# timweiland/DiffEqGMRFs.jl

Measured on AMD Instinct MI355X. Metric: GMRF posterior solves/sec (mean+samples), 256^2 Darcy, higher is better.
Workload: dtype f64; 1 GPU; darcy256: n=65536, 64 blocks x 1024, nnz=1624084; 256 independent posterior(s) per GPU and step (4 stream(s) x batch 64), each factor + mean + 64 samples; mode=problems, samples_per_problem_per_rank=64, l_blocks_kept=False

## Files before the change

diffeqgmrfs.jl_amd/_cabi.py:

```python
from __future__ import annotations

import ctypes as C
import os
from typing import Optional

_HERE = os.path.dirname(os.path.abspath(__file__))
LIB_PATH = os.environ.get("GMRF_HIP_LIBRARY") or os.path.join(_HERE, "csrc", "libgmrf_hip.so")

GMRF_OK = 0
ERR_NOT_SPD, ERR_BAD_SHAPE, ERR_BAND, ERR_HIP, ERR_NO_FACTOR, ERR_NO_DEVICE, ERR_ALLOC, ERR_RCCL = -1, -2, -3, -4, -5, -6, -7, -8
SOLVE_FULL, SOLVE_FORWARD, SOLVE_BACKWARD = 0, 1, 2
VAR_EXACT, VAR_RBMC, VAR_MC = 0, 1, 2
BLOCK_L, BLOCK_C, BLOCK_LINV = 0, 1, 2
ORDER_REFERENCE, ORDER_TWISTED = 0, 1

EXPORTS = [
    "gmrf_bt_create", "gmrf_bt_destroy", "gmrf_last_error", "gmrf_version",
    "gmrf_bt_factor_csc", "gmrf_bt_factor_blocks", "gmrf_bt_refactor_values",
    "gmrf_bt_solve", "gmrf_bt_sample", "gmrf_bt_posterior", "gmrf_bt_set_factor_rhs", "gmrf_bt_normals", "gmrf_bt_marginal_var",
    "gmrf_bt_var_accumulate", "gmrf_bt_logdet", "gmrf_bt_get_block", "gmrf_bt_factor_buffer",
    "gmrf_bt_adopt_shape", "gmrf_bt_adopt_commit", "gmrf_bt_adopt_layout", "gmrf_bt_get_layout", "gmrf_bt_block_range",
    "gmrf_bt_set_keep_l", "gmrf_bt_storage_bytes", "gmrf_bt_set_storage", "gmrf_bt_factor_begin_csc",
    "gmrf_bt_factor_step_async", "gmrf_bt_factor_end", "gmrf_bt_stats",
    "gmrf_bt_set_profiling", "gmrf_bt_set_eager", "gmrf_bt_synchronize", "gmrf_bt_set_batch", "gmrf_bt_select_problem",
    "gmrf_bt_marginal_var_batch", "gmrf_bt_selinv", "gmrf_bt_trace_inv", "gmrf_bt_set_order", "gmrf_bt_get_order", "gmrf_bt_half_stats", "gmrf_bt_export_size", "gmrf_bt_export_factor", "gmrf_bt_import_factor",
    "gmrf_comm_unique_id", "gmrf_comm_create", "gmrf_comm_destroy", "gmrf_comm_bcast_host", "gmrf_comm_allreduce_sum",
    "gmrf_bt_bcast_blocks_async", "gmrf_bt_allgather_blocks_async", "gmrf_comm_wait", "gmrf_comm_bytes", "gmrf_streams_create", "gmrf_streams_destroy",
    "gmrf_bt_packed_size", "gmrf_bt_pack_blocks_async", "gmrf_bt_unpack_blocks_async",
    "gmrf_csr_create", "gmrf_csr_destroy", "gmrf_spmm", "gmrf_spmm_rows", "gmrf_spmm_async", "gmrf_spmm_rows_async",
    "gmrf_darcy_p1_create", "gmrf_darcy_p2_create", "gmrf_darcy_p1_destroy", "gmrf_darcy_p1_pattern", "gmrf_darcy_p1_assemble",
    "gmrf_burgers_p1_create", "gmrf_burgers_p2_create", "gmrf_burgers_line_create", "gmrf_burgers_colloc_create", "gmrf_burgers_p1_destroy", "gmrf_burgers_p1_pattern", "gmrf_burgers_p1_tangent",
    "gmrf_shallow_water_p1_create", "gmrf_shallow_water_p1_destroy", "gmrf_shallow_water_p1_pattern", "gmrf_shallow_water_p1_qpoints",
    "gmrf_shallow_water_p1_assemble", "gmrf_shallow_water_p1_operators",
    "gmrf_assemble_create", "gmrf_assemble_destroy", "gmrf_assemble_pattern", "gmrf_assemble_precision", "gmrf_assemble_rhs",
    "gmrf_burgers_p1_tangent_batch", "gmrf_assemble_precision_batch", "gmrf_assemble_rhs_batch", "gmrf_assemble_objective_batch",
    "gmrf_gn_create", "gmrf_gn_destroy", "gmrf_gn_run", "gmrf_gn_finalize",
    "gmrf_elliptic_p1_create", "gmrf_elliptic_p2_create", "gmrf_elliptic_p1_destroy", "gmrf_elliptic_p1_pattern", "gmrf_elliptic_p1_qpoints",
    "gmrf_elliptic_p1_tangent", "gmrf_elliptic_p1_tangent_batch", "gmrf_elliptic_p1_load", "gmrf_gn_create_elliptic",
    "gmrf_darcy_p1_assemble_batch", "gmrf_dc_create", "gmrf_dc_destroy", "gmrf_dc_run",
    "gmrf_burgers_prior_create", "gmrf_burgers_line_prior_create", "gmrf_burgers_prior_destroy", "gmrf_burgers_prior_pattern", "gmrf_burgers_prior_values_batch",
    "gmrf_bic_create", "gmrf_bic_destroy", "gmrf_bic_run", "gmrf_field_errors_batch",
    "gmrf_test_gemm", "gmrf_test_gemm_desc", "gmrf_test_gemm_pair", "gmrf_test_gemm_rate", "gmrf_test_gemm_shapes", "gmrf_test_potrf_tile", "gmrf_test_potrf_block", "gmrf_test_potrf_route", "gmrf_test_tile_timing", "gmrf_test_persist_stamps", "gmrf_test_persist_aborts", "gmrf_test_factor_fwd", "gmrf_test_gn_route", "gmrf_test_dc_route", "gmrf_test_bic_route", "gmrf_test_var_groups", "gmrf_test_persist_budget", "gmrf_test_clock_probe_start", "gmrf_test_clock_probe_finish",
    "gmrf_test_mfma_f64_rate", "gmrf_test_hbm_rate", "gmrf_test_microbench", "gmrf_test_symbolic_csc",
]


class SparseBlock(C.Structure):
    _fields_ = [("nnz", C.c_int64), ("ptr", C.c_void_p), ("idx", C.c_void_p), ("val", C.c_void_p)]


class Stats(C.Structure):
    _fields_ = [
        ("factor_ms", C.c_double), ("solve_ms", C.c_double), ("sample_ms", C.c_double),
        ("factor_flops", C.c_double), ("sweep_bytes", C.c_double), ("sweep_ms", C.c_double),
        ("n", C.c_int64), ("n_blocks", C.c_int64), ("block_size", C.c_int64),
        ("block_size_padded", C.c_int64), ("factor_bytes", C.c_int64),
        ("kernel_ms", C.c_double * 24), ("kernel_work", C.c_double * 24), ("kernel_launches", C.c_int64 * 24),
        ("sweep_bytes_streamed", C.c_double),
        ("persist_route", C.c_int32), ("persist_aborts", C.c_int32), ("persist_cus", C.c_int32), ("persist_refused", C.c_int32),
        ("sweep_persist", C.c_int32), ("sweep_persist_launches", C.c_int32),
    ]


class GmrfError(RuntimeError):
    def __init__(self, status: int, msg: str, info: int = 0):
        super().__init__(f"libgmrf_hip status {status}: {msg}")
        self.status = status
        self.info = info


class NotPositiveDefinite(GmrfError):
    """Julia's PosDefException(info): `.info` is the failing block (1-based)."""


_lib: Optional[C.CDLL] = None


def load() -> C.CDLL:
    global _lib
    if _lib is not None:
        return _lib
    if not os.path.exists(LIB_PATH):
        raise ImportError(
            f"{LIB_PATH} is missing: build it with `python -c 'import __graft_entry__ as g; g.build()'` "
            "or `make -C diffeqgmrfs.jl_amd/csrc` (the HIP library is the only compute path)")
    try:
        import torch
    except Exception:
        pass
    lib = C.CDLL(LIB_PATH)
    vp, i32, i64, u64, dbl = C.c_void_p, C.c_int32, C.c_int64, C.c_uint64, C.c_double
    P = C.POINTER
    sigs = {
        "gmrf_bt_create": [i32, vp, P(vp)],
        "gmrf_bt_destroy": [vp],
        "gmrf_version": [],
        "gmrf_bt_factor_csc": [vp, i64, i64, vp, vp, vp, i32, P(i32)],
        "gmrf_bt_factor_blocks": [vp, i64, i64, vp, vp, i32, i32, P(i32)],
        "gmrf_bt_refactor_values": [vp, vp, P(i32)],
        "gmrf_bt_solve": [vp, vp, vp, i64, i64, i64, i32],
        "gmrf_bt_sample": [vp, u64, i64, i64, vp, vp, vp, i64],
        "gmrf_bt_posterior": [vp, vp, u64, i64, i64, vp, vp, i64],
        "gmrf_bt_set_factor_rhs": [vp, vp],
        "gmrf_bt_normals": [vp, u64, i64, i64, vp, i64],
        "gmrf_bt_marginal_var": [vp, i32, i64, u64, vp, vp],
        "gmrf_bt_var_accumulate": [vp, i32, i64, i64, u64, vp, vp],
        "gmrf_bt_logdet": [vp, P(dbl)],
        "gmrf_bt_get_block": [vp, i32, i64, vp, i64],
        "gmrf_bt_factor_buffer": [vp, i32, P(vp), P(i64)],
        "gmrf_bt_adopt_shape": [vp, i64, i64],
        "gmrf_bt_storage_bytes": [i64, i64, i64, P(i64), P(i64), P(i64)],
        "gmrf_bt_set_storage": [vp, i64, i64, i64, vp, vp, vp],
        "gmrf_bt_adopt_commit": [vp, i32],
        "gmrf_bt_adopt_layout": [vp, i64, i64, vp, i64],
        "gmrf_bt_get_layout": [vp, vp, i64, P(i64)],
        "gmrf_bt_block_range": [vp, i32, i64, i64, P(i64), P(i64), P(i64)],
        "gmrf_bt_set_keep_l": [vp, i32],
        "gmrf_comm_unique_id": [vp],
        "gmrf_comm_create": [i32, i32, i32, vp, P(vp)],
        "gmrf_comm_destroy": [vp],
        "gmrf_comm_bcast_host": [vp, vp, i64, i32],
        "gmrf_comm_allreduce_sum": [vp, vp, vp, i64],
        "gmrf_bt_bcast_blocks_async": [vp, vp, i32, i64, i64, i32],
        "gmrf_bt_allgather_blocks_async": [vp, vp, vp, i64, i64],
        "gmrf_comm_wait": [vp, vp],
        "gmrf_comm_bytes": [vp, i32, P(dbl)],
        "gmrf_bt_packed_size": [vp, i64, i64, P(i64)],
        "gmrf_bt_pack_blocks_async": [vp, i64, i64, vp],
        "gmrf_bt_unpack_blocks_async": [vp, i64, i64, vp],
        "gmrf_streams_create": [i32, i32, vp, vp],
        "gmrf_streams_destroy": [i32, i32, vp],
        "gmrf_bt_factor_begin_csc": [vp, i64, i64, vp, vp, vp, i32],
        "gmrf_bt_factor_step_async": [vp, i64, i64],
        "gmrf_bt_factor_end": [vp, P(i32)],
        "gmrf_bt_stats": [vp, P(Stats)],
        "gmrf_bt_set_order": [vp, i32, i64],
        "gmrf_bt_get_order": [vp, P(i32), P(i64)],
        "gmrf_bt_half_stats": [vp, i32, P(Stats)],
        "gmrf_bt_set_profiling": [vp, i32],
        "gmrf_bt_set_eager": [vp, i32],
        "gmrf_bt_synchronize": [vp],
        "gmrf_bt_set_batch": [vp, i64],
        "gmrf_bt_select_problem": [vp, i64],
        "gmrf_csr_create": [i32, vp, i64, i64, vp, vp, vp, i32, i32, P(vp)],
        "gmrf_bt_marginal_var_batch": [vp, i32, i64, u64, vp, vp, vp],
        "gmrf_bt_selinv": [vp, vp, vp],
        "gmrf_bt_trace_inv": [vp, vp, vp, i64, vp],
        "gmrf_bt_export_size": [vp, P(i64)],
        "gmrf_bt_export_factor": [vp, vp, i64],
        "gmrf_bt_import_factor": [vp, vp, i64],
        "gmrf_csr_destroy": [vp],
        "gmrf_assemble_create": [i32, vp, i64, vp, vp, i64, vp, vp, i32, P(vp)],
        "gmrf_assemble_destroy": [vp],
        "gmrf_assemble_pattern": [vp, P(i64), P(i64), vp, vp, i32],
        "gmrf_assemble_precision": [vp, vp, vp, dbl, vp],
        "gmrf_assemble_rhs": [vp, vp, vp, vp, vp, dbl, vp],
# ... 10 lines not shown
        "gmrf_burgers_p1_pattern": [vp, P(i64), vp, vp, i32],
        "gmrf_burgers_p1_tangent": [vp, vp, vp, vp],
        "gmrf_burgers_p1_tangent_batch": [vp, i64, vp, vp, vp],
        "gmrf_assemble_precision_batch": [vp, i64, vp, i64, vp, dbl, vp],
        "gmrf_assemble_rhs_batch": [vp, i64, vp, vp, vp, vp, dbl, vp],
        "gmrf_assemble_objective_batch": [vp, i64, vp, i64, vp, vp, vp, dbl, vp],
        "gmrf_gn_create": [vp, vp, vp, P(vp)],
        "gmrf_gn_create_elliptic": [vp, vp, vp, P(vp)],
        "gmrf_elliptic_p1_create": [i32, vp, i64, i64, P(vp)],
        "gmrf_elliptic_p2_create": [i32, vp, i64, i64, P(vp)],
        "gmrf_elliptic_p1_destroy": [vp],
        "gmrf_elliptic_p1_pattern": [vp, P(i64), vp, vp, i32],
        "gmrf_elliptic_p1_qpoints": [vp, vp],
        "gmrf_elliptic_p1_tangent": [vp, vp, vp, vp],
        "gmrf_elliptic_p1_tangent_batch": [vp, i64, vp, vp, vp],
        "gmrf_elliptic_p1_load": [vp, i64, vp, vp],
        "gmrf_gn_destroy": [vp],
        "gmrf_gn_run": [vp, vp, i64, vp, vp, vp, vp, dbl, dbl, i32, vp, vp, P(i32)],
        "gmrf_gn_finalize": [vp, P(i32)],
        "gmrf_darcy_p1_assemble_batch": [vp, i64, vp, i64, dbl, vp, vp],
        "gmrf_dc_create": [vp, vp, vp, P(vp)],
        "gmrf_dc_destroy": [vp],
        "gmrf_dc_run": [vp, vp, i64, dbl, vp, i64, vp, dbl, i64, u64, i32, i64, u64, vp, vp, vp, vp, P(i32)],
        "gmrf_burgers_prior_create": [i32, vp, i64, i64, dbl, dbl, dbl, P(vp)],
        "gmrf_burgers_line_prior_create": [i32, vp, i64, i64, dbl, dbl, dbl, i32, i32, dbl, dbl, i32, P(vp)],
        "gmrf_burgers_prior_destroy": [vp],
        "gmrf_burgers_prior_pattern": [vp, P(i64), vp, vp, i32],
        "gmrf_burgers_prior_values_batch": [vp, i64, vp, vp, vp, vp],
        "gmrf_bic_create": [vp, vp, vp, P(vp)],
        "gmrf_bic_destroy": [vp],
        "gmrf_bic_run": [vp, vp, vp, vp, vp, vp, P(i32)],
        "gmrf_field_errors_batch": [i32, vp, i64, i64, i64, vp, vp, vp],
        "gmrf_shallow_water_p1_create": [i32, vp, i64, i64, P(vp)],
        "gmrf_shallow_water_p1_destroy": [vp],
        "gmrf_shallow_water_p1_pattern": [vp, i32, P(i64), vp, vp, i32],
        "gmrf_shallow_water_p1_qpoints": [vp, vp],
        "gmrf_shallow_water_p1_assemble": [vp, vp, dbl, dbl, dbl, vp, vp, vp, vp],
        "gmrf_shallow_water_p1_operators": [vp, vp, vp, vp, vp, dbl, dbl, dbl, vp, vp, vp, vp],
        "gmrf_spmm": [vp, vp, vp, i64, i64, i64],
        "gmrf_spmm_async": [vp, vp, vp, i64, i64, i64],
        "gmrf_spmm_rows_async": [vp, vp, vp, i64, i64, i64],
        "gmrf_spmm_rows": [vp, vp, vp, i64, i64, i64],
        "gmrf_test_gemm": [i32, i64, i64, i64, i32, i32, i32, i32, dbl, vp, i64, vp, i64, dbl, vp, i64],
        "gmrf_test_gemm_shapes": [vp, P(dbl), i64, P(i64)],
        "gmrf_test_gemm_desc": [i32, i32, vp, vp] + [vp, i64] * 12 + [P(i32)],
        "gmrf_test_gemm_pair": [i32, i32, i32, vp, vp, vp, vp, vp, vp, vp, vp],
        "gmrf_test_gemm_rate": [i32, i64, i64, i64, i32, i32, i32, i32, i32, i32, P(dbl)],
        "gmrf_test_potrf_tile": [i32, vp, vp, P(i32)],
        "gmrf_test_potrf_block": [i32, i64, vp, vp, P(i32)],
        "gmrf_test_potrf_route": [i32, i64, i32, i32, i64, i32, vp, vp, vp, P(i32), P(i32)],
        "gmrf_test_tile_timing": [vp, i32],
        "gmrf_test_persist_stamps": [vp, i32],
        "gmrf_test_persist_aborts": [vp, vp],
        "gmrf_test_factor_fwd": [vp, vp, vp],
        "gmrf_test_gn_route": [vp, P(i32), P(i32)],
        "gmrf_test_dc_route": [vp, vp],
        "gmrf_test_bic_route": [vp, vp],
        "gmrf_test_var_groups": [vp, vp, vp],
        "gmrf_test_persist_budget": [i32, i32, vp, vp],
        "gmrf_test_clock_probe_start": [i32, i32, i32, P(vp)],
        "gmrf_test_clock_probe_finish": [vp, vp, vp],
        "gmrf_test_mfma_f64_rate": [i32, P(dbl)],
        "gmrf_test_hbm_rate": [i32, i64, P(dbl)],
        "gmrf_test_microbench": [i32, vp, i32],
        "gmrf_test_symbolic_csc": [i64, i64, vp, vp, i32, vp],
    }
    for name, args in sigs.items():
        fn = getattr(lib, name)
        fn.argtypes = args
        fn.restype = i32
    lib.gmrf_last_error.argtypes = []
    lib.gmrf_last_error.restype = C.c_char_p
    _lib = lib
    return lib


def check(status: int, info: int = 0):
    if status == GMRF_OK:
        return
    msg = load().gmrf_last_error().decode(errors="replace")
    if status == ERR_NOT_SPD:
        raise NotPositiveDefinite(status, msg, info)
    raise GmrfError(status, msg, info)


def ptr(a) -> C.c_void_p:
    if a is None:
        return C.c_void_p(0)
    if isinstance(a, int):
        return C.c_void_p(a)
    if hasattr(a, "data_ptr"):
        return C.c_void_p(a.data_ptr())
    return C.c_void_p(a.ctypes.data)
```

diffeqgmrfs.jl_amd/api.py:

```python
from __future__ import annotations

import ctypes as C
from typing import List, Optional, Sequence, Tuple

import numpy as np
import scipy.sparse as sp

from . import _cabi
from ._cabi import GmrfError, NotPositiveDefinite


def _is_torch(x) -> bool:
    return hasattr(x, "data_ptr") and hasattr(x, "device")


def _colmajor(b, n: int):
    if _is_torch(b):
        import torch
        if b.dtype != torch.float64:
            raise TypeError("float64 required")
        if b.dim() == 1:
            if b.shape[0] != n:
                raise ValueError("dimension mismatch")
            return b.contiguous(), 1, n, True
# ... 1001 lines not shown
        store, view = _alloc_like(like if like is not None else np.empty(0), self.N, k, False)
        _cabi.check(self._lib.gmrf_bt_normals(self._h, seed, first_id, k, _cabi.ptr(store), self.N))
        return view

    def normals_batch(self, k: int, seed: int = 0x5EED, first_id: int = 0):
        out = np.empty((self.batch, k, self.N), dtype=np.float64)
        _cabi.check(self._lib.gmrf_bt_normals(self._h, seed, first_id, k, _cabi.ptr(out), self.N))
        return out

    def sample(self, k: int, mean=None, z=None, seed: int = 0x5EED, first_id: int = 0, like=None):
        ref = like if like is not None else (z if z is not None else (mean if mean is not None else np.empty(0)))
        za = None
        if z is not None:
            za, kz, _, _ = _colmajor(z, self.N)
            k = kz
        if mean is not None and not _is_torch(mean):
            mean = np.ascontiguousarray(mean, dtype=np.float64)
        store, view = _alloc_like(ref if _is_torch(ref) else np.empty(0), self.N, k, False)
        _cabi.check(self._lib.gmrf_bt_sample(self._h, seed, first_id, k, _cabi.ptr(mean), _cabi.ptr(za),
                                             _cabi.ptr(store), self.N))
        return view

    def posterior(self, b, k: int, seed: int = 0x5EED, first_id: int = 0):
        if self.batch != 1:
            raise ValueError("posterior(): one problem per handle (use solve_batch / sample_batch for batches)")
        xa, kb, ld, one_d = _colmajor(b, self.N)
        if kb != 1:
            raise ValueError("posterior(): one right-hand side")
        mstore, mview = _alloc_like(xa, self.N, 1, True)
        sstore, sview = _alloc_like(xa, self.N, k, False)
        _cabi.check(self._lib.gmrf_bt_posterior(self._h, _cabi.ptr(xa), seed, first_id, k, _cabi.ptr(mstore), _cabi.ptr(sstore),
                                                self.N))
        return mview, sview

    def posterior_batch(self, b, k: int, seed: int = 0x5EED, first_id: int = 0):
        import torch
        B, n = self.batch, self.N
        b = b.reshape(B, n).contiguous()
        mean = torch.empty((B, n), dtype=torch.float64, device=b.device)
        out = torch.empty((B, k, n), dtype=torch.float64, device=b.device)
        _cabi.check(self._lib.gmrf_bt_posterior(self._h, _cabi.ptr(b), seed, first_id, k, _cabi.ptr(mean), _cabi.ptr(out), n))
        return mean, out

    def set_factor_rhs(self, b):
        if b is None:
            self._factor_rhs = None
            _cabi.check(self._lib.gmrf_bt_set_factor_rhs(self._h, None))
            return
        if not (_is_torch(b) and b.is_cuda and b.is_contiguous()) or (self.N and b.numel() != self.batch * self.N):
            raise ValueError("set_factor_rhs(): a contiguous device tensor of batch x n values")
        self._factor_rhs = b
        _cabi.check(self._lib.gmrf_bt_set_factor_rhs(self._h, _cabi.ptr(b)))

    def marginal_var(self, method: str = "exact", k: int = 50, seed: int = 0x5EED, Q: Optional[CsrMatrix] = None,
                     q_values=None, out=None):
        m = {"exact": _cabi.VAR_EXACT, "rbmc": _cabi.VAR_RBMC, "mc": _cabi.VAR_MC}[method]
        shape = (self.N,) if self.batch == 1 else (self.batch, self.N)
        if out is None:
            out = np.empty(shape, dtype=np.float64)
        else:
            ok = tuple(out.shape) == shape and (out.is_contiguous() and str(out.dtype) == "torch.float64" if _is_torch(out)
                                                else out.flags.c_contiguous and out.dtype == np.float64)
            if not ok:
                raise ValueError(f"out must be a contiguous float64 array of shape {shape}")
        if self.batch > 1 and m != _cabi.VAR_EXACT:
            qv = None
            if q_values is not None:
                qv = q_values.contiguous() if _is_torch(q_values) else np.ascontiguousarray(q_values, dtype=np.float64)
            _cabi.check(self._lib.gmrf_bt_marginal_var_batch(self._h, m, k, seed, Q._h if Q is not None else None,
                                                             _cabi.ptr(qv) if qv is not None else None, _cabi.ptr(out)))
            return out
        _cabi.check(self._lib.gmrf_bt_marginal_var(self._h, m, k, seed, Q._h if Q is not None else None,
                                                   _cabi.ptr(out)))
        return out

    def selected_inverse(self, S: CsrMatrix, out=None):
        shape = (S.nnz,) if self.batch == 1 else (self.batch, S.nnz)
        given = out is not None
        out = self._out_array(out, shape)
        _cabi.check(self._lib.gmrf_bt_selinv(self._h, S._h, _cabi.ptr(out)))
        if given or self.batch > 1:
            return out
        return sp.csr_matrix((out, S.indices.copy(), S.indptr.copy()), shape=S.shape)

    def trace_inv(self, S: CsrMatrix, dvals):
        nd = 2 if self.batch == 1 else 3
        if dvals.ndim != nd or dvals.shape[-1] != S.nnz or (nd == 3 and dvals.shape[0] != self.batch):
            want = "(m, nnz)" if nd == 2 else "(batch, m, nnz)"
            raise ValueError(f"dvals must be {want} with nnz = {S.nnz}")
        m = int(dvals.shape[-2])
        if _is_torch(dvals):
            import torch
            if dvals.dtype != torch.float64:
                raise TypeError("float64 required")
            dvals = dvals.contiguous()
            out = torch.empty(dvals.shape[:-1], dtype=torch.float64, device=dvals.device)
        else:
            dvals = np.ascontiguousarray(dvals, dtype=np.float64)
            out = np.empty(dvals.shape[:-1], dtype=np.float64)
        _cabi.check(self._lib.gmrf_bt_trace_inv(self._h, S._h, _cabi.ptr(dvals), m, _cabi.ptr(out)))
        return out

    @staticmethod
    def _out_array(out, shape):
        if out is None:
            return np.empty(shape, dtype=np.float64)
# ... 261 lines not shown
```

diffeqgmrfs.jl_amd/csrc/gmrf_hip.hip:

```cpp
#include <hip/hip_runtime.h>
#include <dlfcn.h>
#include <stdint.h>
#include <stdlib.h>
#include <string.h>
#include <time.h>

#include <algorithm>
#include <atomic>
#include <iterator>
#include <cmath>
#include <map>
#include <memory>
#include <chrono>
#include <functional>
#include <initializer_list>
#include <mutex>
#include <string>
#include <type_traits>
#include <vector>

#include "../../include/gmrf_hip.h"
#include "assemble.hpp"
#include "fem_assemble.hpp"
#include "burgers_line.hpp"
// ... 138 lines not shown
    int64_t lo_row_max = 0;
    bool sparse_b = false;
    bool dense_g1 = false;
    double *d_L = nullptr, *d_C = nullptr, *d_Linv = nullptr;
    bool external_storage = false;
    bool keep_l = true;
    bool l_valid = false;
    bool logdet_valid = false;
    std::vector<char> got_block;
    int64_t alloc_rm = 0, alloc_wc = 0;
    bool alloc_keep_l = true;
    double *d_S = nullptr, *d_B = nullptr, *d_T = nullptr, *d_W = nullptr;
    double* d_V = nullptr;
    int64_t v_elems = 0;
    uint64_t layout_gen = 0;
    uint64_t sel_csr = 0, sel_gen = ~0ull;
    int64_t sel_nnz = 0;
    std::vector<int64_t> sel_off, sel_nd;
    int64_t* d_sel_src = nullptr;
    int64_t* d_sel_slot = nullptr;
    int64_t sel_cap = 0;
    double* d_sig = nullptr;
    int64_t sig_elems = 0;
    double* d_dv = nullptr;
    int64_t dv_elems = 0;
    int* d_info = nullptr;
    double* d_logdet = nullptr;
    int64_t alloc_N = 0, alloc_bsp = 0;
    bool factored = false;
    double *d_P = nullptr, *d_Y = nullptr, *d_Tp = nullptr;
    int64_t kp_cap = 0;
    double* d_stage = nullptr;
    int64_t stage_cap = 0;
    DevBuf mean_arena;
    double* d_acc = nullptr;
    int64_t acc_B = 0;
    int32_t var_group = 0, var_groups = 0;
    bool eager = false;
    bool split_step = false;
    bool sweep_no_gemm = false;
    bool no_fused_posterior = false;
    bool tail_probe = false;
    bool tail_refused = false;
    const double* frhs = nullptr;
    const double* fy_for = nullptr;
    bool fwd_run = false;
    bool no_factor_fwd = false;
    bool no_grouped_gemm = false;
    GemmDirectOut* d_dout = nullptr;
    double* d_ft = nullptr;
    double* d_fy = nullptr;
    int64_t fy_elems = 0;
    const double* factor_graph_rhs = nullptr;
    unsigned long long* dbg_stamps = nullptr;
    bool fork_graph = false;
    bool no_staircase = false;
    bool doubling_x = false;
    int xsplit = 0;
    int adopt_xsplit = 0;
    bool no_xsplit = false;
    bool no_lookahead = false;
    bool no_persist = false;
    bool persist_gave_up = false;
    bool persist_launched = false;
    int persist_cus = 0;
    int info_checked = 0;
    int factor_graph_route = 0;
    int persist_aborts = 0;
    int cu_count = 0;
    unsigned* d_pflags = nullptr;
    int64_t pflags_words = 0;
    bool no_sweep_persist = false;
    bool no_scatter_fold = false;
    bool sweep_persist_planned = false;
    bool sweep_persist_launched = false;
    unsigned* d_sweep_flags = nullptr;
    double* d_Tsw = nullptr;
    int64_t t_elems = 0;
    unsigned* h_sweep_abort = nullptr;
    int sweep_nw = 0;
    double *d_P2 = nullptr, *d_Y2 = nullptr, *d_T2 = nullptr;
    int64_t p2_elems = 0;
    bool sweep_persist_hold = false;
    bool no_persist_panels = false;
    hipStream_t aux = nullptr;
    bool aux_distinct = false;
    hipStream_t gemm_stream = nullptr;
    bool capturing = false;
    std::vector<hipEvent_t> fork_events;
    size_t fork_next = 0;
    hipGraphExec_t factor_graph = nullptr;
    int64_t factor_graph_i0 = -1, factor_graph_i1 = -1;
    std::map<int64_t, hipGraphExec_t> sweep_graphs;
    int profiling = 0;
    std::vector<EvPair> events;
    std::vector<hipEvent_t> ev_pool;
    std::vector<GemmShapeStat> gemm_shapes;
    gmrf_stats stats;
    hipEvent_t ev0 = nullptr, ev1 = nullptr;
    int order = GMRF_ORDER_REFERENCE;
    int64_t meet_req = -1;
    int32_t eager_bits = 0;
    TwistState* tw = nullptr;
    int64_t tw_blk = -1;
    const double* tw_hj = nullptr;
    double* tw_w = nullptr;
// ... 311 lines not shown
    HIPCHK(hipMalloc(&h->d_S, blk));
    HIPCHK(hipMalloc(&h->d_B, blk));
    HIPCHK(hipMalloc(&h->d_T, blk));
    HIPCHK(hipMalloc(&h->d_W, blk));
    HIPCHK(hipMalloc(&h->d_logdet, sizeof(double) * h->N * h->B));
    {
        const int64_t words = (int64_t)persist_flag_words((int)(h->bsp / 64)) * h->B;
        if (!h->d_pflags || h->pflags_words < words) {
            free_dev(h->d_pflags); h->d_pflags = nullptr; h->pflags_words = 0;
            HIPCHK(hipMalloc(&h->d_pflags, sizeof(unsigned) * (size_t)words));
            HIPCHK(hipMemsetAsync(h->d_pflags, 0, sizeof(unsigned) * (size_t)words, h->stream));
            HIPCHK(hipStreamSynchronize(h->stream));
            h->pflags_words = words;
        }
    }
    h->alloc_N = h->N; h->alloc_bsp = h->bsp; h->alloc_B = h->B;
    h->stats.factor_bytes = (int64_t)(blk * ((h->keep_l ? 2 : 1) * h->N) + (size_t)stride_pC(h) * sizeof(double) * (size_t)h->B);
    return GMRF_OK;
}

static void release_shape_buffers(gmrf_handle* h) {
    for (auto& kv : h->sweep_graphs) (void)hipGraphExecDestroy(kv.second);
    h->sweep_graphs.clear();
    free_dev(h->d_P); free_dev(h->d_Y); free_dev(h->d_Tp);
    h->d_P = h->d_Y = h->d_Tp = nullptr; h->kp_cap = 0;
    h->mean_arena.release();
    free_dev(h->d_acc); h->d_acc = nullptr; h->acc_B = 0;
    free_dev(h->d_stage); h->d_stage = nullptr; h->stage_cap = 0;
    free_dev(h->d_ft); free_dev(h->d_fy); h->d_ft = h->d_fy = nullptr; h->fy_elems = 0; h->fy_for = nullptr;
}

static gmrf_status set_shape(gmrf_handle* h, int64_t n, int64_t N) {
    if (n <= 0 || N <= 0 || n % N != 0) return bad_shape("n must be a positive multiple of N_blocks");
    const int64_t bs = n / N;
    if (bs > (1 << 20)) return bad_shape("block size too large");
    if (h->n != n || h->N != N) {
        (void)hipStreamSynchronize(h->stream);
        destroy_graphs(h);
        release_shape_buffers(h);
        h->factored = false;
        h->analyzed = false;
    }
    h->n = n; h->N = N; h->bs = bs;
    h->layout_gen++;
    h->bsp = 64 * next_pow2((bs + 63) / 64);
    h->n_pad = h->bsp * N;
    h->stats.n = n; h->stats.n_blocks = N; h->stats.block_size = bs; h->stats.block_size_padded = h->bsp;
    h->stats.factor_flops = ((double)N * bs * bs * bs / 3.0 + (double)(N - 1) * 2.0 * bs * bs * bs) * (double)h->B;
    return GMRF_OK;
}

static gmrf_status ensure_panels(gmrf_handle* h, int64_t kp) {
    if (kp <= h->kp_cap && h->d_P) return GMRF_OK;
    for (auto& kv : h->sweep_graphs) (void)hipGraphExecDestroy(kv.second);
    h->sweep_graphs.clear();
    free_dev(h->d_P); free_dev(h->d_Y); free_dev(h->d_Tp);
    h->d_P = h->d_Y = h->d_Tp = nullptr;
    HIPCHK(hipMalloc(&h->d_P, sizeof(double) * kp * h->n_pad * h->B));
    HIPCHK(hipMalloc(&h->d_Y, sizeof(double) * kp * h->n_pad * h->B));
    HIPCHK(hipMalloc(&h->d_Tp, sizeof(double) * kp * h->bsp * h->B));
    h->kp_cap = kp;
    return GMRF_OK;
}

static gmrf_status ensure_stage(gmrf_handle* h, int64_t elems) {
    if (elems <= h->stage_cap && h->d_stage) return GMRF_OK;
    free_dev(h->d_stage);
    h->d_stage = nullptr;
    HIPCHK(hipMalloc(&h->d_stage, sizeof(double) * elems));
    h->stage_cap = elems;
    return GMRF_OK;
}

struct HostEntry { uint64_t key; int64_t src; };

struct SymbolicPlan {
    std::vector<int64_t> diag_first, diag_count, low_first, low_count;
    std::vector<uint64_t> keys;
    std::vector<int64_t> src;
    int64_t cmin = 0, rmax = 0;
    std::vector<int64_t> first;
    std::vector<int> rowptr;
    int64_t max_row = 0;
    bool sparse_b = false, bxt_ok = false;
    std::vector<int> uptr, ucols, gtiles, ng;
    std::vector<uint16_t> lidx;
    int ecap = 0, nrt = 0;
    std::vector<int> drowptr;
};

static void build_symbolic(int64_t N, int64_t bsp, const std::vector<std::vector<HostEntry>>& dg,
                           const std::vector<std::vector<HostEntry>>& lo, bool no_staircase, SymbolicPlan& sp, bool group_tiles = true) {
    sp.diag_first.assign((size_t)N, 0); sp.diag_count.assign((size_t)N, 0);
    sp.low_first.assign((size_t)N, 0); sp.low_count.assign((size_t)N, 0);
    auto& keys = sp.keys; auto& src = sp.src;
    keys.clear(); src.clear();
    for (int64_t i = 0; i < N; ++i) {
        sp.diag_first[i] = (int64_t)keys.size(); sp.diag_count[i] = (int64_t)dg[i].size();
        {
            std::vector<HostEntry> drow(dg[i]);
            std::stable_sort(drow.begin(), drow.end(), [](const HostEntry& x, const HostEntry& y) { return x.key < y.key; });
            for (auto& e : drow) { keys.push_back(e.key); src.push_back(e.src); }
        }
        sp.low_first[i] = (int64_t)keys.size(); sp.low_count[i] = (int64_t)lo[i].size();
        std::vector<HostEntry> byrow(lo[i]);
        std::stable_sort(byrow.begin(), byrow.end(), [](const HostEntry& x, const HostEntry& y) { return x.key < y.key; });
// ... 340 lines not shown
        }
    }
    h->sweep_persist_planned = ok && want_s > 0 && want >= want_s;
    const int got = ok ? want : 0;
    if (got != h->persist_cus) destroy_graphs(h);
    h->persist_cus = got;
    h->stats.persist_cus = got;
    h->stats.persist_refused = (want > 0 && !ok) ? 1 : 0;
}
static void persist_release(gmrf_handle* h) {
    std::lock_guard<std::mutex> lock(g_persist_mu);
    auto it = g_persist_claims.find(h->device);
    if (it != g_persist_claims.end()) it->second.erase(h);
    h->persist_cus = 0;
    h->stats.persist_cus = 0;
    h->sweep_persist_planned = false;
}

static void persist_give_up(gmrf_handle* h) {
    h->persist_gave_up = true; h->persist_aborts++;
    h->stats.persist_aborts = h->persist_aborts;
    persist_release(h);
    destroy_graphs(h);
}

static bool persist_fits(const gmrf_handle* h, int nt, int j0, int j1, int xrows) {
    if (h->no_persist || h->persist_gave_up || h->persist_cus <= 0) return false;
    return (int64_t)(1 + persist_tiles(nt, j0, j1, xrows)) * h->B <= h->persist_cus;
}

static gmrf_status launch_persist(gmrf_handle* h, double* S, double* L, double* X, int nt, int j0, int j1, int xrows, int blk_id,
                                  double flops) {
    const int words = persist_flag_words(nt);
    if (!h->d_pflags || h->pflags_words < (int64_t)words * h->B) return bad_shape("internal: flag words of the persistent launches not allocated");
    PersistArgs pa;
    pa.S = S; pa.L = L; pa.X = X; pa.ld = h->bsp; pa.nt = nt; pa.j0 = j0; pa.j1 = j1; pa.xrows = xrows;
    pa.tail_panel = (!xrows && j1 < nt) ? 1 : 0;
    pa.info = h->d_info; pa.blk = blk_id;
    pa.pS = h->bsp * h->bsp; pa.pL = stride_pL(h); pa.pX = stride_pX(h); pa.blk_per_problem = (int)h->N;
    pa.flags = h->d_pflags; pa.flag_stride = words;
    pa.abort_word = reinterpret_cast<unsigned*>(h->d_info + 1);
    static const int limit_ms = [] { const char* e = getenv("GMRF_PERSIST_SPIN_MS"); return e ? atoi(e) : -1; }();
    pa.spin_limit = (unsigned)(limit_ms >= 0 ? limit_ms : (h->B > 1 ? 200 : 2000)) * 100000u;
    pa.stamps = h->dbg_stamps;
    h->persist_launched = true;
    h->stats.persist_route = xrows == 1 ? 1 : (xrows == 0 ? 2 : 3);
    ProfScope ps(h, 17, flops);
    hipLaunchKernelGGL(potrf_persist<false>, dim3(1 + persist_tiles(nt, j0, j1, xrows), (unsigned)h->B), dim3(POTRF_PERSIST_THREADS), POTRF_PERSIST_LDS,
                       h->stream, pa);
    HIPCHK(hipGetLastError());
    return GMRF_OK;
}

static gmrf_status potrf_block(gmrf_handle* h, double* S, double* L, double* X, double* T, int blk_id, double* fy = nullptr) {
    const int bsp = (int)h->bsp;
    const int64_t ld = bsp;
    const int nt = bsp / 64;
    const int route = potrf_route(h);
    const bool fused = route == ROUTE_FUSED;
    if (h->xsplit > 0 && route != ROUTE_PANELS256) return bad_shape("internal: split inverse planned off the 256-column panel route");
    static const int pw_env = [] { const char* e = getenv("GMRF_PANEL_TILES"); return e ? atoi(e) : 4; }();
    const int pw = (!fused && nt >= 8) ? ((pw_env == 2 || pw_env == 8) ? pw_env : 4) : nt;
    const bool fused_in_panel = route == ROUTE_BIG_ONE;
    const bool overlap = h->capturing && h->fork_graph && nt >= 8;
    if (overlap && !h->aux) HIPCHK(hipStreamCreateWithFlags(&h->aux, hipStreamNonBlocking));
    hipEvent_t ev_fork = nullptr, ev_join = nullptr;
    if (overlap) { GCHK(fork_event(h, &ev_fork)); GCHK(fork_event(h, &ev_join)); }
    if (fused && !h->no_lookahead && !h->doubling_x && !overlap && nt >= 2 && persist_fits(h, nt, 0, nt, 1)) {
        const double t3 = 64.0 * 64.0 * 64.0;
        double fl = t3 / 3.0 * nt;
        for (int j = 0; j + 1 < nt; ++j) {
            const int m = nt - j - 1;
            fl += (double)m * t3 + 2.0 * t3 * (m * (m + 1) / 2) + 2.0 * t3 * (0.5 * (double)(j + 1) * (j + 2) + 0.625 * (j + 1));
        }
        return launch_persist(h, S, L, X, nt, 0, nt, 1, blk_id, fl);
    }
    if (fused && !h->no_lookahead && !h->doubling_x && !overlap && nt >= 2) {
        StepArgs sa;
        sa.S = S; sa.L = L; sa.X = X; sa.ld = ld; sa.nt = nt; sa.cend = nt;
        sa.info = h->d_info; sa.blk = blk_id; sa.dbg = nullptr;
        sa.pS = (int64_t)bsp * bsp; sa.pL = stride_pL(h); sa.pX = stride_pX(h); sa.blk_per_problem = (int)h->N;
        const double t3 = 64.0 * 64.0 * 64.0;
        {
            sa.j = 0; sa.lookahead = 0; sa.xrow = -1;
            ProfScope ps(h, 1, t3 / 3.0);
            hipLaunchKernelGGL(potrf_step<false>, dim3(1, 1), dim3(256), POTRF_TILE_LDS, h->stream, sa);
        }
        for (int j = 0; j + 1 < nt; ++j) {
            const int m = nt - j - 1, ntile_wg = m * (m + 1) / 2;
            sa.j = j; sa.lookahead = 1;
            sa.xrow = (j >= 1) ? j : -1; sa.xrow_first = ntile_wg;
            const int nx_wg = (j >= 1) ? 4 * j : 0;
            const double f_x = (j >= 1) ? 2.0 * t3 * (0.5 * (double)j * (j + 1) + 0.625 * j) : 0.0;
            ProfScope ps(h, 1, t3 / 3.0 + (double)m * t3 + 2.0 * t3 * ntile_wg + f_x);
            hipLaunchKernelGGL(potrf_step<false>, dim3(ntile_wg + nx_wg, 1), dim3(256), POTRF_STEP_LDS, h->stream, sa);
        }
        {
            sa.j = nt - 1; sa.lookahead = 0; sa.xrow = nt - 1; sa.xrow_first = 0;
            ProfScope ps(h, 1, 2.0 * t3 * (0.5 * (double)(nt - 1) * nt + 0.625 * (nt - 1)));
            hipLaunchKernelGGL(potrf_step<false>, dim3(4 * (nt - 1), 1), dim3(256), 64 * 18 * sizeof(double), h->stream, sa);
        }
        HIPCHK(hipGetLastError());
        return GMRF_OK;
    }
    if (fy && (route != ROUTE_PANELS256 || overlap)) return bad_shape("internal: forward solve planned off the 256-column panel route");
    if (route == ROUTE_PANELS256 && !overlap) {
        StepArgs sa;
        sa.S = S; sa.L = L; sa.X = X; sa.ld = ld; sa.nt = nt; sa.cend = nt;
        sa.info = h->d_info; sa.blk = blk_id; sa.dbg = nullptr;
        sa.pS = (int64_t)bsp * bsp; sa.pL = stride_pL(h); sa.pX = stride_pX(h); sa.blk_per_problem = (int)h->N;
        const int64_t pW = (int64_t)bsp * bsp;
        const double t3 = 64.0 * 64.0 * 64.0, nb = (double)h->B;
        auto diag128 = [&](int j) -> gmrf_status {
            sa.j = j;
            ProfScope ps(h, 16, (2.0 * t3 / 3.0 + 4.0 * 2.0 * t3 * 0.625) * nb);
            static const size_t lds_pad = [] { const char* e = getenv("GMRF_DIAG128_LDS_PAD_KB"); return (size_t)(e ? atoi(e) : 0) * 1024; }();
            static const bool fat = [] { const char* e = getenv("GMRF_DIAG128_FAT"); return e && atoi(e) != 0; }();
            if (fat) hipLaunchKernelGGL(potrf_diag128, dim3(1, (unsigned)h->B), dim3(256), POTRF_DIAG128_LDS + lds_pad, h->stream, sa);
            else hipLaunchKernelGGL(potrf_diag128_slim, dim3(1, (unsigned)h->B), dim3(256), POTRF_DIAG128_SLIM_LDS + lds_pad, h->stream, sa);
            HIPCHK(hipGetLastError());
            return GMRF_OK;
        };
        static const bool no_small = [] { const char* e = getenv("GMRF_PERSIST_PANELS"); return e && atoi(e) == 0; }();
        const bool persist_panels = !no_small && !h->no_persist_panels && persist_fits(h, 4, 0, 4, 2);
        for (int j = 0; j < nt; j += 4) {
            const int64_t oa = (int64_t)j * 64, ob = oa + 128, oc = oa + 256;
            if (persist_panels) {
                const double fl = (4.0 * t3 / 3.0 + 2.0 * t3 * (6.0 * 0.625 + 10.0 + 10.0 + 6.0 * 0.625)) * nb;
                GCHK(launch_persist(h, S + oa * ld + oa, L + oa * ld + oa, X + oa * ld + oa, 4, 0, 4, 2, blk_id, fl));
            } else {
                GCHK(diag128(j));
                GCHK(gemm(h, false, false, 128, 128, 128, TRI_B_UPPER, 0, 1.0, S + ob * ld + oa, ld, X + oa * ld + oa, ld, 0.0, L + ob * ld + oa, ld,
                          sa.pS, sa.pX, sa.pL, 1, 0, 0, 0, nullptr, 0, 0, 0, 2.0 * t3 * 3.0 * 2.0 * nb));
                GCHK(gemm_pair(h,
                               GemmOne{false, 128, 128, 128, 0, 1, -1.0, L + ob * ld + oa, ld, L + ob * ld + oa, ld, 1.0, S + ob * ld + ob, ld,
                                       sa.pL, sa.pL, sa.pS, 2.0 * t3 * 2.0 * 3.0 * nb},
                               GemmOne{true, 128, 128, 128, TRI_B_LOWER, 0, 1.0, L + ob * ld + oa, ld, X + oa * ld + oa, ld, 0.0, T + ob * ld + oa, ld,
                                       sa.pL, sa.pX, pW, -1.0}));
                GCHK(diag128(j + 2));
                GCHK(gemm(h, false, true, 128, 128, 128, TRI_A_LOWER, 0, -1.0, X + ob * ld + ob, ld, T + ob * ld + oa, ld, 0.0, X + ob * ld + oa, ld,
                          sa.pX, pW, sa.pX));
            }
            const int m3 = nt - j - 4;
            const int64_t pT = bsp, pY = h->n_pad;
            if (m3 <= 0) {
                if (fy) {
                    SweepArgs sw;
                    sw.Mat = X + oa * ld + oa; sw.ld = ld; sw.Xin = h->d_ft + oa; sw.ldx = pT; sw.Bin = nullptr; sw.ldb = 0;
                    sw.Out = fy + oa; sw.ldo = pY; sw.rows = 256; sw.kdim = 256; sw.sub = 0;
                    sw.pMat = sa.pX; sw.pXin = pT; sw.pBin = 0; sw.pOut = pY;
                    ProfScope ps(h, 3, 4.0 * 256.0 * 257.0 * nb);
                    HIPCHK(launch_sweep(h->stream, false, true, 1, sw, (int)h->B));
                }
                continue;
            }
            const GemmTail tp{h->d_ft + oa, pT, fy + oa, pY, nullptr, 0, 0.0};
            const GemmTail tu{fy + oa, pY, h->d_ft + oc, pT, nullptr, 0, 1.0};
            const bool in_slot = (j == 0 && h->xsplit == 256 && !h->keep_l);
            double* Lb = in_slot ? X + oc * ld + oa : L + oc * ld + oa;
            const int64_t pLb = in_slot ? sa.pX : sa.pL;
            GCHK(gemm(h, false, false, 64 * m3, 256, 256, TRI_B_UPPER, 0, 1.0, S + oc * ld + oa, ld, X + oa * ld + oa, ld, 0.0, Lb, ld,
                      sa.pS, sa.pX, pLb, 1, 0, 0, 0, nullptr, 0, 0, 0, 2.0 * t3 * 10.0 * m3 * nb, nullptr, nullptr, nullptr, false,
                      fy ? &tp : nullptr));
            GCHK(gemm(h, false, false, m3 * 64, m3 * 64, 256, 0, 1, -1.0, Lb, ld, Lb, ld, 1.0, S + oc * ld + oc, ld, pLb, pLb, sa.pS,
                      1, 0, 0, 0, nullptr, 0, 0, 0, 2.0 * t3 * 4.0 * (m3 * (m3 + 1) / 2) * nb, nullptr, nullptr, nullptr, false,
                      fy ? &tu : nullptr));
        }
        const int p = h->xsplit;
        GCHK(doubling_levels(h, L, X, T, 256, bsp / 2, -1, p));
        if (p > 0 && !(p == 256 && !h->keep_l)) {
            hipLaunchKernelGGL(copy_rect, dim3((unsigned)((bsp - p) / 4), (unsigned)h->B), dim3(256), 0, h->stream,
                               L + (int64_t)p * ld, ld, sa.pL, X + (int64_t)p * ld, ld, sa.pX, bsp - p, p);
            HIPCHK(hipGetLastError());
        }
        return GMRF_OK;
    }
    if (h->xsplit > 0) return bad_shape("internal: split inverse planned off the 256-column panel route");
// ... 227 lines not shown
    const int bsp = (int)h->bsp, p = h->xsplit, q = bsp - p;
    const int64_t ld = bsp, bstride = (int64_t)bsp * bsp, pX = stride_pX(h), pW = bstride;
    for (int64_t i = 0; i < h->N; ++i) {
        double* X = h->d_Linv + i * bstride;
        double* T = h->d_T + (int64_t)p * ld;
        GCHK(gemm(h, false, true, q, p, p, TRI_B_LOWER, 0, 1.0, X + (int64_t)p * ld, ld, X, ld, 0.0, T, ld, pX, pX, pW));
        GCHK(gemm(h, false, true, q, p, q, TRI_A_LOWER, 0, -1.0, X + (int64_t)p * ld + p, ld, T, ld, 0.0, X + (int64_t)p * ld, ld, pX, pW, pX));
    }
    h->xsplit = 0;
    return GMRF_OK;
}

static std::mutex g_capture_mu;

static gmrf_status factor_fwd_ok(gmrf_handle* h, bool* ok) {
    *ok = false;
    if (!h->frhs || h->no_factor_fwd || h->B <= 1 || tw_on(h) || h->tw_blk >= 0 || h->fork_graph || h->rmax <= 0) return GMRF_OK;
    const int bsp = (int)h->bsp, nt = bsp / 64;
    if (potrf_route(h) != ROUTE_PANELS256 || bsp % 256 != 0) return GMRF_OK;
    const int64_t elems = h->B * h->n_pad + h->B * h->bsp;
    if (!h->d_fy || h->fy_elems < elems) {
        HIPCHK(hipStreamSynchronize(h->stream));
        free_dev(h->d_ft); free_dev(h->d_fy); h->d_ft = h->d_fy = nullptr; h->fy_elems = 0; h->fy_for = nullptr;
        HIPCHK(hipMalloc(&h->d_fy, sizeof(double) * (size_t)(h->B * h->n_pad)));
        HIPCHK(hipMalloc(&h->d_ft, sizeof(double) * (size_t)(h->B * h->bsp)));
        h->fy_elems = elems;
    }
    const int64_t ld = bsp, bstride = (int64_t)bsp * bsp, pX = stride_pX(h), pL = stride_pL(h), pC = stride_pC(h);
    const int cm = (int)h->cmin, rm = (int)h->rmax, W = bsp - cm;
    double* S = h->d_S; double* X = h->d_Linv; double* L = h->d_L;
    h->tail_probe = true; h->tail_refused = false;
    gmrf_status st = GMRF_OK;
    if (h->N > 1) {
        const GemmTail tg{h->d_fy + cm, h->n_pad, h->d_ft, bsp, nullptr, 0, 1.0};
        st = gemm(h, false, false, rm, rm, W, 0, 1, -1.0, h->d_C, c_ld(h), h->d_C, c_ld(h), 0.0, S, ld, pC, pC, bstride, 1, 0, 0, 0,
                  nullptr, 0, 0, 0, -1.0, h->d_kst, h->d_kst, nullptr, false, &tg);
    }
    for (int j = 0; j + 4 < nt && st == GMRF_OK; j += 4) {
        const int64_t oa = (int64_t)j * 64, oc = oa + 256;
        const int m3 = nt - j - 4;
        const GemmTail tp{h->d_ft + oa, bsp, h->d_fy + oa, h->n_pad, nullptr, 0, 0.0};
        const GemmTail tu{h->d_fy + oa, h->n_pad, h->d_ft + oc, bsp, nullptr, 0, 1.0};
        st = gemm(h, false, false, 64 * m3, 256, 256, TRI_B_UPPER, 0, 1.0, S + oc * ld + oa, ld, X + oa * ld + oa, ld, 0.0, L + oc * ld + oa, ld,
                  bstride, pX, pL, 1, 0, 0, 0, nullptr, 0, 0, 0, -1.0, nullptr, nullptr, nullptr, false, &tp);
        if (st == GMRF_OK)
            st = gemm(h, false, false, m3 * 64, m3 * 64, 256, 0, 1, -1.0, L + oc * ld + oa, ld, L + oc * ld + oa, ld, 1.0, S + oc * ld + oc, ld,
                      pL, pL, bstride, 1, 0, 0, 0, nullptr, 0, 0, 0, -1.0, nullptr, nullptr, nullptr, false, &tu);
    }
    h->tail_probe = false;
    *ok = st == GMRF_OK && !h->tail_refused;
    return GMRF_OK;
}

static gmrf_status run_factor(gmrf_handle* h, int64_t i0, int64_t i1) {
    if (h->eager || h->profiling) { h->stats.persist_route = 0; return factor_blocks_range(h, i0, i1); }
    const double* grhs = h->fwd_run ? h->frhs : nullptr;
    if (!h->factor_graph || h->factor_graph_i0 != i0 || h->factor_graph_i1 != i1 || h->factor_graph_rhs != grhs) {
        std::lock_guard<std::mutex> capture_lock(g_capture_mu);
        if (h->factor_graph) { (void)hipGraphExecDestroy(h->factor_graph); h->factor_graph = nullptr; }
        hipGraph_t graph = nullptr;
        HIPCHK(hipStreamBeginCapture(h->stream, hipStreamCaptureModeThreadLocal));
        h->capturing = true; h->fork_next = 0;
        h->stats.persist_route = 0;
        gmrf_status s = factor_blocks_range(h, i0, i1);
        h->capturing = false;
        h->factor_graph_route = h->stats.persist_route;
        hipError_t e = hipStreamEndCapture(h->stream, &graph);
        if (s != GMRF_OK) { if (graph) (void)hipGraphDestroy(graph); return s; }
        HIPCHK(e);
        HIPCHK(hipGraphInstantiate(&h->factor_graph, graph, nullptr, nullptr, 0));
        (void)hipGraphDestroy(graph);
        h->factor_graph_i0 = i0; h->factor_graph_i1 = i1; h->factor_graph_rhs = grhs;
    }
    h->xsplit = planned_xsplit(h);
    h->stats.persist_route = h->factor_graph_route;
    if (h->factor_graph_route) h->persist_launched = true;
    HIPCHK(hipGraphLaunch(h->factor_graph, h->stream));
    return GMRF_OK;
}

static gmrf_status persist_check_range(gmrf_handle* h, int64_t i0, int64_t i1, int* hinfo_out) {
    int hinfo2[2] = {0, 0};
    HIPCHK(hipMemcpyAsync(hinfo2, h->d_info, 2 * sizeof(int), hipMemcpyDeviceToHost, h->stream));
    HIPCHK(hipStreamSynchronize(h->stream));
    h->persist_launched = false;
    if (hinfo2[1] != 0) {
        persist_give_up(h);
        const int restore[4] = {h->info_checked, 0, 0, 0};
        HIPCHK(hipMemcpyAsync(h->d_info, restore, 4 * sizeof(int), hipMemcpyHostToDevice, h->stream));
        if (h->d_pflags) HIPCHK(hipMemsetAsync(h->d_pflags, 0, sizeof(unsigned) * (size_t)h->pflags_words, h->stream));
        h->stats.persist_route = 0;
        GCHK(factor_blocks_range(h, i0, i1));
        HIPCHK(hipMemcpyAsync(hinfo2, h->d_info, 2 * sizeof(int), hipMemcpyDeviceToHost, h->stream));
        HIPCHK(hipStreamSynchronize(h->stream));
        h->persist_launched = false;
    }
    h->info_checked = hinfo2[0];
    if (hinfo_out) *hinfo_out = hinfo2[0];
    return GMRF_OK;
}

static gmrf_status factor_finish(gmrf_handle* h, int32_t* info) {
    int hinfo = 0;
    GCHK(persist_check_range(h, 0, h->N, &hinfo));
    if (info) *info = hinfo;
    if (hinfo != 0) {
        h->factored = false;
        g_last_error = "matrix is not positive definite; failed block " + std::to_string((hinfo - 1) % h->N + 1) +
                       " of problem " + std::to_string((hinfo - 1) / h->N);
        if (info) *info = (hinfo - 1) % (int)h->N + 1;
        return GMRF_ERR_NOT_SPD;
    }
    h->factored = true;
    h->l_valid = h->keep_l;
    h->logdet_valid = !h->keep_l;
    return GMRF_OK;
}

static gmrf_status numeric_factor(gmrf_handle* h, const double* nzval, int32_t* info) {
    if (!h->analyzed) { g_last_error = "no sparsity pattern analysed"; return GMRF_ERR_NO_FACTOR; }
    GCHK(alloc_factor(h));
    if (h->c_dirty) {
        HIPCHK(hipMemsetAsync(h->d_C, 0, sizeof(double) * stride_pC(h) * h->B, h->stream));
        h->c_dirty = false;
    }
    persist_plan(h);
    HIPCHK(hipEventRecord(h->ev0, h->stream));
    GCHK(load_values(h, nzval));
    HIPCHK(hipMemsetAsync(h->d_info, 0, 4 * sizeof(int), h->stream));
    h->info_checked = 0; h->persist_launched = false;
    h->fy_for = nullptr;
    bool fwd = false;
    GCHK(factor_fwd_ok(h, &fwd));
    h->fwd_run = fwd;
    gmrf_status s = run_factor(h, 0, h->N);
    if (s == GMRF_OK) {
        (void)hipEventRecord(h->ev1, h->stream);
        s = factor_finish(h, info);
    }
    h->fwd_run = false;
    if (s == GMRF_OK && fwd) h->fy_for = h->frhs;
    float ms = 0.f;
    (void)hipEventElapsedTime(&ms, h->ev0, h->ev1);
    h->stats.factor_ms = ms;
    if (h->profiling) prof_collect(h);
    return s;
}

__global__ void gmrf_spin_kernel(unsigned long long ticks) {
    const unsigned long long t0 = __builtin_amdgcn_s_memrealtime();
    while (__builtin_amdgcn_s_memrealtime() - t0 < ticks) {}
}

static double spin_pair_ms(hipStream_t a, hipStream_t b, unsigned long long ticks) {
    (void)hipDeviceSynchronize();
    const auto t0 = std::chrono::steady_clock::now();
    hipLaunchKernelGGL(gmrf_spin_kernel, dim3(1), dim3(64), 0, a, ticks);
    if (b) hipLaunchKernelGGL(gmrf_spin_kernel, dim3(1), dim3(64), 0, b, ticks);
    (void)hipStreamSynchronize(a);
    if (b) (void)hipStreamSynchronize(b);
    return std::chrono::duration<double, std::milli>(std::chrono::steady_clock::now() - t0).count();
}

gmrf_status gmrf_streams_create(int32_t device, int32_t n, void** streams, int32_t* n_distinct) {
    if (n <= 0 || n > 32 || !streams) return bad_shape("gmrf_streams_create: 1 <= n <= 32 streams");
    HIPCHK(hipSetDevice(device));
    const int ncand = std::min(3 * n + 4, 48);
    std::vector<hipStream_t> cand((size_t)ncand, nullptr);
    for (int i = 0; i < ncand; ++i) {
        if (hipStreamCreateWithFlags(&cand[(size_t)i], hipStreamNonBlocking) != hipSuccess) {
            for (int j = 0; j < i; ++j) (void)hipStreamDestroy(cand[(size_t)j]);
            g_last_error = "hipStreamCreateWithFlags failed"; return GMRF_ERR_HIP;
        }
        hipLaunchKernelGGL(gmrf_spin_kernel, dim3(1), dim3(64), 0, cand[(size_t)i], 1ull);
    }
    HIPCHK(hipDeviceSynchronize());
    const unsigned long long ticks = 100000ull;
    double one = 1e30;
    for (int r = 0; r < 3; ++r) one = std::min(one, spin_pair_ms(cand[0], nullptr, ticks));
    std::vector<int> chosen;
    for (int i = 0; i < ncand && (int)chosen.size() < n; ++i) {
        bool ok = true;
        for (int c : chosen) {
            const double t = std::min(spin_pair_ms(cand[(size_t)c], cand[(size_t)i], ticks), spin_pair_ms(cand[(size_t)c], cand[(size_t)i], ticks));
            if (t > 1.5 * one) { ok = false; break; }
        }
        if (ok) chosen.push_back(i);
    }
    const int nd = (int)chosen.size();
    std::vector<char> used((size_t)ncand, 0);
    for (int c : chosen) used[(size_t)c] = 1;
    for (int i = 0; i < ncand && (int)chosen.size() < n; ++i)
        if (!used[(size_t)i]) { chosen.push_back(i); used[(size_t)i] = 1; }
    for (int k = 0; k < n; ++k) streams[k] = (void*)cand[(size_t)chosen[(size_t)k]];
// ... 163 lines not shown
        double* yout = Yout + i * bsp;
        auto direct = [&](int first) { return GemmTail{nullptr, 0, nullptr, 0, nullptr, 0, 0.0, dout, i * h->bs + first, (int)h->bs - first}; };
        if (h->xsplit > 0) {
            const int p = h->xsplit, q = bsp - p;
            const double* Xbb = X + (int64_t)p * ld + p;
            const double* Lba = X + (int64_t)p * ld;
            for (int part = 0; part < 3; ++part) {
                const int which = backward ? 2 - part : part;
                if (via_gemm) {
                    constexpr int64_t z0 = 0;
                    const GemmTail da = direct(0), db = direct(p);
                    if (which == 0)
                        GCHK(gemm(h, false, backward, kp, p, p, backward ? TRI_B_LOWER : TRI_B_UPPER, 0, 1.0, rhs, npad, X, ld, 0.0, yout, npad,
                                  pPanel, pX, pPanel, 1, z0, z0, z0, nullptr, z0, z0, 0, -1.0, nullptr, nullptr, nullptr, tail,
                                  dout ? &da : nullptr));
                    else if (which == 2)
                        GCHK(gemm(h, false, backward, kp, q, q, backward ? TRI_B_LOWER : TRI_B_UPPER, 0, 1.0, rhs + p, npad, Xbb, ld, 0.0,
                                  yout + p, npad, pPanel, pX, pPanel, 1, z0, z0, z0, nullptr, z0, z0, 0, -1.0, nullptr, nullptr, nullptr, tail,
                                  dout ? &db : nullptr));
                    else if (!backward)
                        GCHK(gemm(h, false, false, kp, q, p, 0, 0, -1.0, yout, npad, Lba, ld, 1.0, rhs + p, npad, pPanel, pX, pPanel));
                    else
                        GCHK(gemm(h, false, true, kp, p, q, 0, 0, -1.0, yout + p, npad, Lba, ld, 1.0, rhs, npad, pPanel, pX, pPanel,
                                  1, z0, z0, z0, nullptr, z0, z0, 0, -1.0, nullptr, nullptr, nullptr, tail));
                } else {
                    s.ld = ld; s.ldx = npad; s.ldo = npad; s.pMat = pX; s.pXin = pPanel; s.pOut = pPanel; s.kst = nullptr; s.mend = nullptr;
                    if (which == 0) { s.Mat = X; s.Xin = rhs; s.Bin = nullptr; s.ldb = 0; s.Out = yout; s.rows = p; s.kdim = p; s.sub = 0; s.pBin = 0; }
                    else if (which == 2) { s.Mat = Xbb; s.Xin = rhs + p; s.Bin = nullptr; s.ldb = 0; s.Out = yout + p; s.rows = q; s.kdim = q; s.sub = 0; s.pBin = 0; }
                    else if (!backward) { s.Mat = Lba; s.Xin = yout; s.Bin = rhs + p; s.ldb = npad; s.Out = rhs + p; s.rows = q; s.kdim = p; s.sub = 1; s.pBin = pPanel; }
                    else { s.Mat = Lba; s.Xin = yout + p; s.Bin = rhs; s.ldb = npad; s.Out = rhs; s.rows = p; s.kdim = q; s.sub = 1; s.pBin = pPanel; }
                    const double frac = which == 0 ? (double)p * (p + 1) : (which == 2 ? (double)q * (q + 1) : 2.0 * p * q);
                    ProfScope ps(h, pclass, blk_work_t * frac / ((double)bsp * (bsp + 1)));
                    HIPCHK(launch_sweep(h->stream, backward, which != 1, kp, s, nprob));
                }
            }
        } else if (via_gemm) {
            const GemmTail da = direct(0);
            GCHK(gemm(h, false, backward, kp, bsp, bsp, backward ? TRI_B_LOWER : TRI_B_UPPER, 0, 1.0, rhs, npad, X, ld, 0.0,
                      yout, npad, pPanel, pX, pPanel, 1, 0, 0, 0, nullptr, 0, 0, 0, -1.0, nullptr, nullptr, nullptr, tail, dout ? &da : nullptr));
        } else {
            s.Mat = X; s.ld = ld; s.Xin = rhs; s.ldx = npad; s.Bin = nullptr; s.ldb = 0; s.Out = yout; s.ldo = npad;
            s.rows = bsp; s.kdim = bsp; s.sub = 0;
            s.pMat = pX; s.pXin = pPanel; s.pBin = 0; s.pOut = pPanel;
            s.kst = nullptr; s.mend = nullptr;
            ProfScope ps(h, pclass, blk_work_t);
            HIPCHK(launch_sweep(h->stream, backward, true, kp, s, nprob));
        }
    }
    return GMRF_OK;
}

constexpr int SWEEP_BACKWARD_YP = 3, SWEEP_BACKWARD_TAIL = 4;
static gmrf_status run_sweeps(gmrf_handle* h, int mode, int kp) {
    auto body = [&]() -> gmrf_status {
        if (mode == GMRF_SOLVE_FORWARD) return sweep_launches(h, false, kp, h->d_P, h->d_Y);
        if (mode == SWEEP_BACKWARD_TAIL) return sweep_launches(h, true, kp, h->d_P, h->d_Y, true, h->d_dout);
        if (mode == SWEEP_BACKWARD_YP) return sweep_launches(h, true, kp, h->d_Y, h->d_P);
        if (mode == GMRF_SOLVE_BACKWARD) return sweep_launches(h, true, kp, h->d_P, h->d_Y);
        GCHK(sweep_launches(h, false, kp, h->d_P, h->d_Y));
        return sweep_launches(h, true, kp, h->d_Y, h->d_P);
    };
    const bool persistent = mode != SWEEP_BACKWARD_TAIL && sweep_persist_ok(h, kp);
    if (persistent) {
        GCHK(sweep_persist_prepare(h, kp));
        h->sweep_persist_launched = true;
        h->stats.sweep_persist = 1;
        h->stats.sweep_persist_launches += (mode == GMRF_SOLVE_FULL) ? 2 : 1;
    }
    if (h->eager || h->profiling) return body();
    const int64_t key = ((int64_t)h->xsplit << 32) | ((int64_t)mode * 4096 + kp) |
                        (persistent ? ((int64_t)1 << 60) : 0);
    auto it = h->sweep_graphs.find(key);
    if (it == h->sweep_graphs.end()) {
        std::lock_guard<std::mutex> capture_lock(g_capture_mu);
        hipGraph_t graph = nullptr;
        hipGraphExec_t exec = nullptr;
        HIPCHK(hipStreamBeginCapture(h->stream, hipStreamCaptureModeThreadLocal));
        gmrf_status s = body();
        hipError_t e = hipStreamEndCapture(h->stream, &graph);
        if (s != GMRF_OK) { if (graph) (void)hipGraphDestroy(graph); return s; }
        HIPCHK(e);
        HIPCHK(hipGraphInstantiate(&exec, graph, nullptr, nullptr, 0));
        (void)hipGraphDestroy(graph);
        it = h->sweep_graphs.emplace(key, exec).first;
    }
    HIPCHK(hipGraphLaunch(it->second, h->stream));
    return GMRF_OK;
}

static int pad_k(int64_t k) { return k == 1 ? 1 : (int)((k + 15) / 16 * 16); }

static gmrf_status launch_pack(gmrf_handle* h, const double* d_src, int64_t ld, int k, int kp) {
    const int64_t total = (int64_t)kp * h->n_pad;
    hipLaunchKernelGGL(pack_panel, dim3((unsigned)((total + 255) / 256), (unsigned)h->B), dim3(256), 0, h->stream, d_src, ld,
                       h->d_P, h->n_pad, (int)h->bs, (int)h->bsp, (int)h->N, k, kp);
    HIPCHK(hipGetLastError());
    return GMRF_OK;
}

static gmrf_status launch_unpack(gmrf_handle* h, const double* panel, double* d_dst, int64_t ld, int k,
                                 const double* d_mean) {
    const int64_t total = h->n * (int64_t)k;
    hipLaunchKernelGGL(unpack_panel, dim3((unsigned)((total + 255) / 256), (unsigned)h->B), dim3(256), 0, h->stream, panel,
                       h->n_pad, d_dst, ld, (int)h->bs, (int)h->bsp, h->n, k, pad_k(k), d_mean);
    HIPCHK(hipGetLastError());
    return GMRF_OK;
}

static gmrf_status cols_in(gmrf_handle* h, const double* src, int64_t ld, bool src_dev, int k, const double** d_src, int64_t* d_ld) {
    *d_src = src; *d_ld = ld;
    if (src_dev) return GMRF_OK;
    GCHK(ensure_stage(h, (int64_t)k * h->n * h->B));
    HIPCHK(hipMemcpy2DAsync(h->d_stage, h->n * sizeof(double), src, ld * sizeof(double),
                            h->n * sizeof(double), k * h->B, hipMemcpyHostToDevice, h->stream));
    *d_src = h->d_stage; *d_ld = h->n;
    return GMRF_OK;
}

static gmrf_status cols_out(gmrf_handle* h, const double* panel, int k, const double* d_mean, double* dst, int64_t ld, bool dst_dev) {
    if (dst_dev) return launch_unpack(h, panel, dst, ld, k, d_mean);
    GCHK(ensure_stage(h, (int64_t)k * h->n * h->B));
    GCHK(launch_unpack(h, panel, h->d_stage, h->n, k, d_mean));
    HIPCHK(hipMemcpy2DAsync(dst, ld * sizeof(double), h->d_stage, h->n * sizeof(double),
                            h->n * sizeof(double), k * h->B, hipMemcpyDeviceToHost, h->stream));
    return GMRF_OK;
}

constexpr int64_t KP_CHUNK = 128;

static void tw_free(gmrf_handle* h);
static gmrf_status tw_analyze(gmrf_handle* h, int64_t n, int64_t N, const int64_t* colptr, const int64_t* rowval, int32_t base);
static gmrf_status tw_numeric(gmrf_handle* h, const double* nzval, int32_t* info);
static gmrf_status tw_solve(gmrf_handle* h, const double* b, double* y, int64_t k, int64_t ldb, int64_t ldy, int mode);
static gmrf_status tw_sample(gmrf_handle* h, uint64_t seed, int64_t first_id, int64_t k, const double* mean, const double* z,
                             double* out, int64_t ld);
static gmrf_status tw_logdet(gmrf_handle* h, double* out);
static gmrf_status tw_get_block(gmrf_handle* h, int32_t kind, int64_t i, double* out, int64_t ld);
static gmrf_status tw_var_exact(gmrf_handle* h, double* d_out);
static gmrf_status tw_var_accumulate_dev(gmrf_handle* h, int method, int64_t first_id, int64_t k, uint64_t seed, const gmrf_csr* Q,
                                         double* d_acc);

extern "C" {

int32_t gmrf_version(void) { return 100; }
const char* gmrf_last_error(void) { return g_last_error.c_str(); }

gmrf_status gmrf_bt_create(int32_t device, void* stream, gmrf_handle** out) {
    if (!out) return bad_shape("null out pointer");
    int count = 0;
    if (hipGetDeviceCount(&count) != hipSuccess || count <= 0 || device < 0 || device >= count) {
        (void)hipGetLastError();
        g_last_error = "no HIP device visible (libgmrf_hip needs an MI355X / gfx950 GPU)";
        return GMRF_ERR_NO_DEVICE;
    }
    HIPCHK(hipSetDevice(device));
    gmrf_handle* h = new gmrf_handle();
    memset(&h->stats, 0, sizeof(h->stats));
    h->device = device;
    if (stream) { h->stream = (hipStream_t)stream; h->own_stream = false; }
    else { HIPCHK(hipStreamCreateWithFlags(&h->stream, hipStreamNonBlocking)); h->own_stream = true; }
    HIPCHK(hipMalloc(&h->d_info, 4 * sizeof(int)));
    HIPCHK(hipMemsetAsync(h->d_info, 0, 4 * sizeof(int), h->stream));
    HIPCHK(hipStreamSynchronize(h->stream));
    HIPCHK(hipEventCreate(&h->ev0));
    HIPCHK(hipEventCreate(&h->ev1));
    HIPCHK(hipFuncSetAttribute((const void*)potrf_step<false>, hipFuncAttributeMaxDynamicSharedMemorySize, (int)POTRF_STEP_LDS));
    HIPCHK(hipFuncSetAttribute((const void*)potrf_diag128, hipFuncAttributeMaxDynamicSharedMemorySize, 160 * 1024));
    HIPCHK(hipFuncSetAttribute((const void*)potrf_persist<false>, hipFuncAttributeMaxDynamicSharedMemorySize, (int)POTRF_PERSIST_LDS));
    HIPCHK(hipDeviceGetAttribute(&h->cu_count, hipDeviceAttributeMultiprocessorCount, device));
    { const char* e = getenv("GMRF_PERSIST"); if (e && atoi(e) == 0) h->no_persist = true; }
    { const char* e = getenv("GMRF_SWEEP_PERSIST"); if (e && atoi(e) == 0) h->no_sweep_persist = true; }
    HIPCHK(hipFuncSetAttribute((const void*)potrf_diag128_slim, hipFuncAttributeMaxDynamicSharedMemorySize, 160 * 1024));
    HIPCHK(gemm_init());
    HIPCHK(gemm_dma_init());
    *out = h;
    return GMRF_OK;
}

gmrf_status gmrf_bt_destroy(gmrf_handle* h) {
    if (!h) return GMRF_OK;
    (void)hipSetDevice(h->device);
    tw_free(h);
    (void)hipStreamSynchronize(h->stream);
    persist_release(h);
    destroy_graphs(h);
    free_dev(h->d_keys); free_dev(h->d_vals); free_dev(h->d_src); free_dev(h->d_nz_stage);
    free_dev(h->d_lo_rowptr); free_dev(h->d_dg_rowptr); free_dev(h->d_kst); free_dev(h->d_mend);
    free_dev(h->d_bxt_uptr); free_dev(h->d_bxt_ucols); free_dev(h->d_bxt_lidx); free_dev(h->d_bxt_gtiles);
    if (!h->external_storage) { free_dev(h->d_L); free_dev(h->d_C); free_dev(h->d_Linv); }
    else if (!h->keep_l) free_dev(h->d_L);
    free_dev(h->d_S); free_dev(h->d_B); free_dev(h->d_T); free_dev(h->d_W);
    free_dev(h->d_sweep_flags); free_dev(h->d_Tsw); free_dev(h->d_P2); free_dev(h->d_Y2); free_dev(h->d_T2);
    if (h->h_sweep_abort) { (void)hipHostFree(h->h_sweep_abort); h->h_sweep_abort = nullptr; }
    free_dev(h->d_dout); free_dev(h->d_info); free_dev(h->d_logdet); free_dev(h->d_pflags); free_dev(h->d_kbx); free_dev(h->d_V);
    free_dev(h->d_P); free_dev(h->d_Y); free_dev(h->d_Tp);
    free_dev(h->d_stage); h->mean_arena.release(); free_dev(h->d_acc);
    free_dev(h->d_ft); free_dev(h->d_fy);
    free_dev(h->d_sel_src); free_dev(h->d_sel_slot); free_dev(h->d_sig); free_dev(h->d_dv);
    for (auto e : h->ev_pool) (void)hipEventDestroy(e);
    if (h->ev0) (void)hipEventDestroy(h->ev0);
    if (h->ev1) (void)hipEventDestroy(h->ev1);
    for (auto e : h->fork_events) (void)hipEventDestroy(e);
    if (h->aux) (void)hipStreamDestroy(h->aux);
    if (h->own_stream) (void)hipStreamDestroy(h->stream);
    delete h;
    return GMRF_OK;
}

gmrf_status gmrf_bt_set_batch(gmrf_handle* h, int64_t batch) {
    if (!h || batch < 1 || batch > 4096) return bad_shape("batch must be in [1, 4096]");
    if (batch != 1) GCHK(tw_refuse(h, "gmrf_bt_set_batch (batch > 1)"));
    if (batch != h->B) {
        HIPCHK(hipSetDevice(h->device));
        HIPCHK(hipStreamSynchronize(h->stream));
        destroy_graphs(h);
        h->B = batch;
        h->sel = 0;
        h->factored = false;
        release_shape_buffers(h);
        if (h->n > 0) (void)set_shape(h, h->n, h->N);
    }
    return GMRF_OK;
}

gmrf_status gmrf_bt_select_problem(gmrf_handle* h, int64_t p) {
    if (!h || p < 0 || p >= h->B) return bad_shape("problem index out of range");
    h->sel = p;
    return GMRF_OK;
}

gmrf_status gmrf_bt_set_profiling(gmrf_handle* h, int32_t level) {
    if (!h) return bad_shape("null handle");
    h->profiling = level;
    if (h->tw)
        for (gmrf_handle* s : {h->tw->top, h->tw->bot}) if (s) GCHK(gmrf_bt_set_profiling(s, level));
    if (level > 0 && h->events.empty()) h->gemm_shapes.clear();
    for (int i = 0; i < GMRF_KERNEL_CLASSES; ++i) { h->stats.kernel_ms[i] = h->stats.kernel_work[i] = 0; h->stats.kernel_launches[i] = 0; }
    return GMRF_OK;
}

gmrf_status gmrf_bt_set_eager(gmrf_handle* h, int32_t eager) {
    if (!h) return bad_shape("null handle");
    if (((eager & 2) != 0) != h->split_step) { destroy_graphs(h); h->split_step = (eager & 2) != 0; }
    if (((eager & 4) != 0) != h->sweep_no_gemm) { destroy_graphs(h); h->sweep_no_gemm = (eager & 4) != 0; }
    if (((eager & 8) != 0) != h->dense_g1) { destroy_graphs(h); h->dense_g1 = (eager & 8) != 0; }
    if (((eager & 16) != 0) != h->fork_graph) { destroy_graphs(h); h->fork_graph = (eager & 16) != 0; }
    h->no_staircase = (eager & 32) != 0;
    if (((eager & 128) != 0) != h->doubling_x) { destroy_graphs(h); h->doubling_x = (eager & 128) != 0; }
    if (((eager & 256) != 0) != h->no_lookahead) { destroy_graphs(h); h->no_lookahead = (eager & 256) != 0; }
    if (((eager & 4096) != 0) != h->no_xsplit) { destroy_graphs(h); h->no_xsplit = (eager & 4096) != 0; }
    if (((eager & 8192) != 0) != h->no_persist) { destroy_graphs(h); h->no_persist = (eager & 8192) != 0; }
    if (((eager & 32768) != 0) != h->no_persist_panels) { destroy_graphs(h); h->no_persist_panels = (eager & 32768) != 0; }
    if (((eager & 65536) != 0) != h->no_sweep_persist) { destroy_graphs(h); h->no_sweep_persist = (eager & 65536) != 0; }
    if (((eager & 131072) != 0) != h->no_scatter_fold) { destroy_graphs(h); h->no_scatter_fold = (eager & 131072) != 0; }
    h->no_fused_posterior = (eager & 262144) != 0;
    h->no_factor_fwd = (eager & 524288) != 0;
    if (((eager & 1048576) != 0) != h->no_grouped_gemm) { destroy_graphs(h); h->no_grouped_gemm = (eager & 1048576) != 0; }
    if (eager != h->eager_bits) h->fy_for = nullptr;
    h->eager = (eager & 1) != 0;
    h->eager_bits = eager;
    if (h->tw)
        for (gmrf_handle* s : {h->tw->top, h->tw->bot})
            if (s) {
                GCHK(gmrf_bt_set_eager(s, eager));
                if (h->tw->bot) s->no_sweep_persist = true;
            }
    return GMRF_OK;
}

gmrf_status gmrf_bt_synchronize(gmrf_handle* h) {
    if (!h) return bad_shape("null handle");
    HIPCHK(hipStreamSynchronize(h->stream));
    if (tw_on(h)) HIPCHK(hipStreamSynchronize(h->tw->bot->stream));
    return GMRF_OK;
}

gmrf_status gmrf_bt_stats(gmrf_handle* h, gmrf_stats* out) {
    if (!h || !out) return bad_shape("null pointer");
    if (tw_on(h)) {
        const gmrf_stats &a = h->tw->top->stats, &b = h->tw->bot->stats;
        *out = h->stats;
        out->persist_route = a.persist_route;
        out->persist_aborts = a.persist_aborts + b.persist_aborts;
        out->persist_cus = a.persist_cus + b.persist_cus;
        out->persist_refused = a.persist_refused | b.persist_refused;
        out->factor_bytes = a.factor_bytes + b.factor_bytes;
        return GMRF_OK;
    }
    h = tw_route(h);
    *out = h->stats;
    return GMRF_OK;
}

gmrf_status gmrf_bt_factor_csc(gmrf_handle* h, int64_t n, int64_t n_blocks, const int64_t* colptr,
                               const int64_t* rowval, const double* nzval, int32_t index_base,
                               int32_t* info) {
    if (!h) return bad_shape("null handle");
    HIPCHK(hipSetDevice(h->device));
    if (info) *info = 0;
    if (h->order == GMRF_ORDER_TWISTED) {
        GCHK(tw_analyze(h, n, n_blocks, colptr, rowval, index_base));
        return tw_numeric(h, nzval, info);
    }
    GCHK(analyze_csc(h, n, n_blocks, colptr, rowval, index_base));
    return numeric_factor(h, nzval, info);
}

gmrf_status gmrf_bt_factor_begin_csc(gmrf_handle* h, int64_t n, int64_t n_blocks, const int64_t* colptr,
                                     const int64_t* rowval, const double* nzval, int32_t index_base) {
    GCHK(tw_refuse(h, "gmrf_bt_factor_begin_csc"));
    if (!h) return bad_shape("null handle");
    HIPCHK(hipSetDevice(h->device));
    if (colptr) GCHK(analyze_csc(h, n, n_blocks, colptr, rowval, index_base));
    if (!h->analyzed) { g_last_error = "no sparsity pattern analysed"; return GMRF_ERR_NO_FACTOR; }
    GCHK(alloc_factor(h));
    if (h->c_dirty) {
        HIPCHK(hipMemsetAsync(h->d_C, 0, sizeof(double) * stride_pC(h) * h->B, h->stream));
        h->c_dirty = false;
    }
    persist_plan(h);
    GCHK(load_values(h, nzval));
    HIPCHK(hipMemsetAsync(h->d_info, 0, 4 * sizeof(int), h->stream));
    h->info_checked = 0; h->persist_launched = false; h->stats.persist_route = 0;
    h->factored = false; h->fy_for = nullptr;
    return GMRF_OK;
}

gmrf_status gmrf_bt_factor_step_async(gmrf_handle* h, int64_t i0, int64_t i1) {
    GCHK(tw_refuse(h, "gmrf_bt_factor_step_async"));
    if (!h) return bad_shape("null handle");
    if (i0 < 0 || i1 > h->N || i0 > i1) return bad_shape("bad block range");
    HIPCHK(hipSetDevice(h->device));
    GCHK(factor_blocks_range(h, i0, i1));
    if (h->persist_launched) GCHK(persist_check_range(h, i0, i1, nullptr));
    return GMRF_OK;
}

gmrf_status gmrf_bt_factor_end(gmrf_handle* h, int32_t* info) {
    GCHK(tw_refuse(h, "gmrf_bt_factor_end"));
    if (!h) return bad_shape("null handle");
    HIPCHK(hipSetDevice(h->device));
    gmrf_status s = factor_finish(h, info);
    if (h->profiling) prof_collect(h);
    return s;
}

gmrf_status gmrf_bt_refactor_values(gmrf_handle* h, const double* nzval, int32_t* info) {
    if (!h) return bad_shape("null handle");
    HIPCHK(hipSetDevice(h->device));
    if (info) *info = 0;
    if (h->order == GMRF_ORDER_TWISTED) return tw_numeric(h, nzval, info);
    return numeric_factor(h, nzval, info);
}

gmrf_status gmrf_bt_factor_blocks(gmrf_handle* h, int64_t n, int64_t n_blocks, const gmrf_sparse_block* diag,
                                  const gmrf_sparse_block* lower, int32_t index_base,
                                  int32_t compressed_by_column, int32_t* info) {
    GCHK(tw_refuse(h, "gmrf_bt_factor_blocks"));
    if (!h || !diag || (n_blocks > 1 && !lower)) return bad_shape("null pointer");
    HIPCHK(hipSetDevice(h->device));
    if (info) *info = 0;
    GCHK(set_shape(h, n, n_blocks));
    const int64_t bs = h->bs;
    std::vector<std::vector<HostEntry>> dg(n_blocks), lo(n_blocks);
    std::vector<double> vals;
    auto add_block = [&](const gmrf_sparse_block& b, std::vector<HostEntry>& dst, bool lower_tri_only) -> bool {
        for (int64_t o = 0; o < bs; ++o) {
            for (int64_t p = b.ptr[o] - index_base; p < b.ptr[o + 1] - index_base; ++p) {
                const int64_t in = b.idx[p] - index_base;
                if (in < 0 || in >= bs) return false;
                const int64_t r = compressed_by_column ? in : o, c = compressed_by_column ? o : in;
                if (lower_tri_only && r < c) continue;
                dst.push_back({((uint64_t)r << 32) | (uint64_t)c, (int64_t)vals.size()});
                vals.push_back(b.val[p]);
            }
        }
        return true;
// ... 75 lines not shown
    for (int64_t t = 0; t < nrt; ++t) out[3 + t] = h->kst[(size_t)t];
    out[3 + nrt] = h->factored ? h->xsplit : planned_xsplit(h);
    return GMRF_OK;
}

gmrf_status gmrf_bt_adopt_layout(gmrf_handle* h, int64_t n, int64_t n_blocks, const int64_t* layout, int64_t count) {
    GCHK(tw_refuse(h, "gmrf_bt_adopt_layout"));
    if (!h) return bad_shape("null handle");
    HIPCHK(hipSetDevice(h->device));
    GCHK(set_shape(h, n, n_blocks));
    h->analyzed = false;
    if (layout) {
        if (count < 3 || layout[2] < 1 || count < 3 + layout[2] || layout[1] != 64 * layout[2]) return bad_shape("bad layout record");
        std::vector<int64_t> first((size_t)layout[2]);
        for (int64_t t = 0; t < layout[2]; ++t) first[(size_t)t] = layout[0] + layout[3 + t];
        GCHK(set_layout(h, layout[0], layout[1], first));
        h->adopt_xsplit = 0;
        if (count >= 4 + layout[2]) {
            const int64_t xs = layout[3 + layout[2]];
            if (xs < 0 || xs >= h->bsp || xs % 64) return bad_shape("bad layout record (split)");
            h->adopt_xsplit = (int)xs;
        }
    } else {
        GCHK(set_layout_dense(h));
        h->adopt_xsplit = 0;
    }
    GCHK(alloc_factor(h));
    if (h->c_dirty) {
        HIPCHK(hipMemsetAsync(h->d_C, 0, sizeof(double) * stride_pC(h) * h->B, h->stream));
        h->c_dirty = false;
    }
    h->factored = false; h->l_valid = false; h->logdet_valid = false;
    h->got_block.assign((size_t)h->N, 0);
    HIPCHK(hipStreamSynchronize(h->stream));
    return GMRF_OK;
}

gmrf_status gmrf_bt_adopt_shape(gmrf_handle* h, int64_t n, int64_t n_blocks) {
    GCHK(tw_refuse(h, "gmrf_bt_adopt_shape"));
    return gmrf_bt_adopt_layout(h, n, n_blocks, nullptr, 0);
}

gmrf_status gmrf_bt_adopt_commit(gmrf_handle* h, int32_t l_blocks_valid) {
    GCHK(tw_refuse(h, "gmrf_bt_adopt_commit"));
    if (!h || !h->d_Linv) return bad_shape("no factor storage");
    HIPCHK(hipSetDevice(h->device));
    int seen = 0;
    HIPCHK(hipMemcpyAsync(&seen, h->d_info + 2, sizeof(int), hipMemcpyDeviceToHost, h->stream));
    HIPCHK(hipStreamSynchronize(h->stream));
    if (seen != 0) HIPCHK(hipMemsetAsync(h->d_info + 2, 0, sizeof(int), h->stream));
    if (seen < 0) { g_last_error = "the packed ranges of this factor carry different (or no) representation tags"; return GMRF_ERR_BAD_SHAPE; }
    const int xs = seen > 0 ? seen - 1 : h->adopt_xsplit;
    if (xs < 0 || xs >= h->bsp || xs % 64) { g_last_error = "bad representation tag in the packed image"; return GMRF_ERR_BAD_SHAPE; }
    h->factored = true; h->fy_for = nullptr;
    h->xsplit = xs;
    h->l_valid = l_blocks_valid != 0 && h->keep_l;
    bool all = !h->got_block.empty();
    for (char g : h->got_block) all = all && g;
    h->logdet_valid = all;
    h->got_block.assign((size_t)h->N, 0);
    persist_plan(h);
    return GMRF_OK;
}

gmrf_status gmrf_bt_factor_buffer(gmrf_handle* h, int32_t kind, void** dev_ptr, int64_t* bytes) {
    GCHK(tw_refuse(h, "gmrf_bt_factor_buffer"));
    if (!h || !dev_ptr || !bytes) return bad_shape("null pointer");
    if (!h->d_Linv) { g_last_error = "no factor storage"; return GMRF_ERR_NO_FACTOR; }
    const int64_t blk = blk_elems(h) * (int64_t)sizeof(double) * h->B;
    if (kind == GMRF_BLOCK_L) {
        if (!h->keep_l) { g_last_error = "L blocks are not kept (gmrf_bt_set_keep_l)"; return GMRF_ERR_NO_FACTOR; }
        *dev_ptr = h->d_L; *bytes = blk * h->N;
    }
    else if (kind == GMRF_BLOCK_C) { *dev_ptr = h->d_C; *bytes = stride_pC(h) * (int64_t)sizeof(double) * h->B; }
    else if (kind == GMRF_BLOCK_LINV) { *dev_ptr = h->d_Linv; *bytes = blk * h->N; }
    else return bad_shape("bad block kind");
    return GMRF_OK;
}

gmrf_status gmrf_bt_block_range(gmrf_handle* h, int32_t kind, int64_t i0, int64_t i1, int64_t* first_elem,
                                int64_t* n_elems, int64_t* problem_stride) {
    GCHK(tw_refuse(h, "gmrf_bt_block_range"));
    if (!h || !first_elem || !n_elems || !problem_stride) return bad_shape("null pointer");
    if (h->N <= 0 || i0 < 0 || i1 > h->N || i0 > i1) return bad_shape("bad block range");
    if (kind == GMRF_BLOCK_C) {
        const int64_t c0 = std::max<int64_t>(i0 - 1, 0), c1 = std::max<int64_t>(i1 - 1, 0);
        *first_elem = c0 * c_blk(h); *n_elems = (c1 - c0) * c_blk(h); *problem_stride = stride_pC(h);
    } else if (kind == GMRF_BLOCK_LINV || kind == GMRF_BLOCK_L) {
        if (kind == GMRF_BLOCK_L && !h->keep_l) { g_last_error = "L blocks are not kept"; return GMRF_ERR_NO_FACTOR; }
        *first_elem = i0 * blk_elems(h); *n_elems = (i1 - i0) * blk_elems(h);
        *problem_stride = kind == GMRF_BLOCK_L ? stride_pL(h) : stride_pX(h);
    } else return bad_shape("bad block kind");
    return GMRF_OK;
}

static void packed_counts(const gmrf_handle* h, int64_t i0, int64_t i1, int64_t* x_elems, int64_t* c_elems, int64_t* ld_elems,
                          int64_t* c0_out) {
    const int64_t nt = h->bsp / 64, ntri = nt * (nt + 1) / 2;
    const int64_t c0 = std::max<int64_t>(i0 - 1, 0), c1 = std::max<int64_t>(i1 - 1, 0);
    *x_elems = (i1 - i0) * ntri * 4096;
    *c_elems = (c1 - c0) * c_blk(h);
    *ld_elems = 2 + ((i1 - i0) + 1) / 2 * 2;
    if (c0_out) *c0_out = c0;
}

gmrf_status gmrf_bt_packed_size(gmrf_handle* h, int64_t i0, int64_t i1, int64_t* elems_per_problem) {
    GCHK(tw_refuse(h, "gmrf_bt_packed_size"));
// ... 133 lines not shown
    for (int64_t i = 0; i < h->N; ++i) GCHK(gmrf_bt_get_block(h, GMRF_BLOCK_LINV, i, out + i * be, h->bs));
    return GMRF_OK;
}

gmrf_status gmrf_bt_import_factor(gmrf_handle* h, const void* buf, int64_t bytes) {
    GCHK(tw_refuse(h, "gmrf_bt_import_factor"));
    if (!h || !buf) return bad_shape("null pointer");
    if (is_device_ptr(buf)) return bad_shape("import buffer must be host memory");
    if (bytes < 64) return bad_shape("import buffer too small");
    const int64_t* hdr = (const int64_t*)buf;
    if (hdr[0] != EXPORT_MAGIC || hdr[1] != 1 || hdr[5] != 1) return bad_shape("not a factor image");
    const int64_t n = hdr[2], N = hdr[3], bs = hdr[4];
    if (N <= 0 || bs <= 0 || n != N * bs) return bad_shape("bad shape in factor image");
    if (bytes < 64 + (int64_t)sizeof(double) * bs * bs * (3 * N - 1)) return bad_shape("factor image truncated");
    HIPCHK(hipSetDevice(h->device));
    if (!h->keep_l) return bad_shape("import needs the L blocks kept (gmrf_bt_set_keep_l(h, 1))");
    if ((h->n != n || h->N != N) && h->B != 1) return bad_shape("a batched handle imports into an existing shape only");
    const bool relayout = (h->n != n || h->N != N || h->cmin != 0 || h->rmax != 64 * next_pow2((bs + 63) / 64) || !h->d_Linv);
    if (relayout && h->B != 1 && h->factored) return bad_shape("a batched handle imports only into a dense-layout factor");
    GCHK(set_shape(h, n, N));
    h->analyzed = false;
    if (relayout) {
        GCHK(set_layout_dense(h));
        GCHK(alloc_factor(h));
        if (h->c_dirty) {
            HIPCHK(hipMemsetAsync(h->d_C, 0, sizeof(double) * stride_pC(h) * h->B, h->stream));
            h->c_dirty = false;
        }
    } else {
        std::vector<int64_t> z((size_t)(h->bsp / 64), 0);
        bool dense_ks = true;
        for (int v : h->kst) if (v != 0) dense_ks = false;
        if (!dense_ks) GCHK(set_layout(h, 0, h->bsp, z));
        h->c_dirty = false;
    }
    const int64_t bsp = h->bsp, be = bs * bs;
    std::vector<double> tmp((size_t)bsp * bsp);
    auto put = [&](const double* src, double* dst, bool unit_pad) -> gmrf_status {
        std::fill(tmp.begin(), tmp.end(), 0.0);
        for (int64_t r = 0; r < bs; ++r)
            for (int64_t c = 0; c < bs; ++c) tmp[(size_t)r * bsp + c] = src[c * bs + r];
        if (unit_pad)
            for (int64_t r = bs; r < bsp; ++r) tmp[(size_t)r * bsp + r] = 1.0;
        HIPCHK(hipMemcpyAsync(dst, tmp.data(), tmp.size() * sizeof(double), hipMemcpyHostToDevice, h->stream));
        HIPCHK(hipStreamSynchronize(h->stream));
        return GMRF_OK;
    };
    const double* in = (const double*)((const char*)buf + 64);
    for (int64_t i = 0; i < N; ++i) GCHK(put(in + i * be, h->d_L + h->sel * stride_pL(h) + i * blk_elems(h), true));
    in += N * be;
    for (int64_t i = 0; i + 1 < N; ++i) GCHK(put(in + i * be, h->d_C + h->sel * stride_pC(h) + i * c_blk(h), false));
    in += (N - 1) * be;
    for (int64_t i = 0; i < N; ++i) GCHK(put(in + i * be, h->d_Linv + h->sel * stride_pX(h) + i * blk_elems(h), true));
    h->factored = true; h->fy_for = nullptr; h->l_valid = true;
    persist_plan(h);
    h->xsplit = 0;
    return GMRF_OK;
}

struct NcclUid { char b[128]; };
struct RcclApi {
    void* lib = nullptr;
    int (*GetUniqueId)(NcclUid*) = nullptr;
    int (*CommInitRank)(void**, int, NcclUid, int) = nullptr;
    int (*CommDestroy)(void*) = nullptr;
    int (*Broadcast)(const void*, void*, size_t, int, int, void*, hipStream_t) = nullptr;
    int (*AllReduce)(const void*, void*, size_t, int, int, void*, hipStream_t) = nullptr;
    int (*AllGather)(const void*, void*, size_t, int, void*, hipStream_t) = nullptr;
    int (*GroupStart)() = nullptr;
    int (*GroupEnd)() = nullptr;
    const char* (*GetErrorString)(int) = nullptr;
};
static RcclApi g_rccl;
static std::mutex g_rccl_mu;

static gmrf_status rccl_load() {
    std::lock_guard<std::mutex> lock(g_rccl_mu);
    if (g_rccl.lib) return GMRF_OK;
    const char* env = getenv("GMRF_RCCL_PATH");
    const char* names[] = {env, "librccl.so.1", "librccl.so", "/opt/rocm/lib/librccl.so.1", "/opt/rocm/lib/librccl.so"};
    void* lib = nullptr;
    for (int pass = 0; pass < 2 && !lib; ++pass)
        for (const char* nm : names) {
            if (!nm) continue;
            lib = dlopen(nm, RTLD_NOW | RTLD_LOCAL | (pass == 0 ? RTLD_NOLOAD : 0));
            if (lib) break;
        }
    if (!lib) { g_last_error = std::string("librccl not found (set GMRF_RCCL_PATH): ") + (dlerror() ? dlerror() : ""); return GMRF_ERR_RCCL; }
#define GMRF_RCCL_SYM(field, name)                                                           \
    g_rccl.field = reinterpret_cast<decltype(g_rccl.field)>(dlsym(lib, name));               \
    if (!g_rccl.field) { g_last_error = std::string("librccl lacks ") + name; return GMRF_ERR_RCCL; }
    GMRF_RCCL_SYM(GetUniqueId, "ncclGetUniqueId") GMRF_RCCL_SYM(CommInitRank, "ncclCommInitRank")
    GMRF_RCCL_SYM(CommDestroy, "ncclCommDestroy") GMRF_RCCL_SYM(Broadcast, "ncclBroadcast")
    GMRF_RCCL_SYM(AllReduce, "ncclAllReduce") GMRF_RCCL_SYM(AllGather, "ncclAllGather") GMRF_RCCL_SYM(GroupStart, "ncclGroupStart")
    GMRF_RCCL_SYM(GroupEnd, "ncclGroupEnd") GMRF_RCCL_SYM(GetErrorString, "ncclGetErrorString")
#undef GMRF_RCCL_SYM
    g_rccl.lib = lib;
    return GMRF_OK;
}

#define NCCLCHK(expr)                                                                       \
    do {                                                                                    \
        int _r = (expr);                                                                    \
        if (_r != 0) {                                                                      \
            g_last_error = std::string(#expr) + ": " + g_rccl.GetErrorString(_r);           \
            return GMRF_ERR_RCCL;                                                           \
        }                                                                                   \
// ... 162 lines not shown
}

gmrf_status gmrf_bt_solve(gmrf_handle* h, const double* b, double* y, int64_t k, int64_t ldb, int64_t ldy, int32_t mode) {
    h = tw_route(h);
    if (!h || !b || !y) return bad_shape("null pointer");
    if (!h->factored) { g_last_error = "solve before factor"; return GMRF_ERR_NO_FACTOR; }
    if (k <= 0 || ldb < h->n || ldy < h->n || mode < 0 || mode > 2) return bad_shape("bad k / ldb / ldy / mode");
    if (b == y && ldb != ldy) return bad_shape("in place (y == b) needs ldb == ldy");
    HIPCHK(hipSetDevice(h->device));
    if (tw_on(h)) return tw_solve(h, b, y, k, ldb, ldy, mode);
    if (h->B > 1 && k > KP_CHUNK) return bad_shape("with a batch of problems k is limited to 128 per call");
    const bool b_dev = is_device_ptr(b), y_dev = is_device_ptr(y);
    const int64_t nb = h->B;
    return sweep_guarded(h, {{b, cols_bytes(h->n, k * nb, ldb), y, cols_bytes(h->n, k * nb, ldy)}}, [&]() -> gmrf_status {
        h->stats.solve_ms = 0.0;
        for (int64_t c0 = 0; c0 < k; c0 += KP_CHUNK) {
            const int kc = (int)std::min<int64_t>(KP_CHUNK, k - c0);
            const int kp = pad_k(kc);
            GCHK(ensure_panels(h, kp));
            const double* d_b = nullptr;
            int64_t ld_b = 0;
            GCHK(cols_in(h, b + c0 * ldb, ldb, b_dev, kc, &d_b, &ld_b));
            GCHK(launch_pack(h, d_b, ld_b, kc, kp));
            HIPCHK(hipEventRecord(h->ev0, h->stream));
            GCHK(run_sweeps(h, mode, kp));
            HIPCHK(hipEventRecord(h->ev1, h->stream));
            GCHK(cols_out(h, (mode == GMRF_SOLVE_FULL) ? h->d_P : h->d_Y, kc, nullptr, y + c0 * ldy, ldy, y_dev));
            HIPCHK(hipStreamSynchronize(h->stream));
            float ms = 0.f;
            (void)hipEventElapsedTime(&ms, h->ev0, h->ev1);
            h->stats.solve_ms += ms;
            const int nsweeps = (mode == GMRF_SOLVE_FULL) ? 2 : 1;
            h->stats.sweep_ms = ms / nsweeps;
            h->stats.sweep_bytes = sweep_bytes(h, kc) * (double)nb;
            h->stats.sweep_bytes_streamed = (8.0 * ((double)h->N * 0.5 * (double)h->bsp * (double)(h->bsp + 1) +
                                                    (double)(h->N - 1) * h->c_streamed) + 16.0 * (double)h->n_pad * kc) * (double)nb;
            if (h->profiling) prof_collect(h);
        }
        return GMRF_OK;
    });
}

static gmrf_status sample_chunk(gmrf_handle* h, uint64_t seed, int64_t first_id, int kc, const double* z,
                                int64_t ldz, int64_t id_stride) {
    const int kp = pad_k(kc);
    GCHK(ensure_panels(h, kp));
    if (z) {
        const double* d_z = nullptr;
        int64_t ldd = 0;
        GCHK(cols_in(h, z, ldz, is_device_ptr(z), kc, &d_z, &ldd));
        GCHK(launch_pack(h, d_z, ldd, kc, kp));
    } else {
        const int64_t total = (int64_t)kp * h->n_pad;
        hipLaunchKernelGGL(fill_normals_panel, dim3((unsigned)((total + 255) / 256), (unsigned)h->B), dim3(256), 0,
                           h->stream, h->d_P, h->n_pad, (int)h->bs, (int)h->bsp, kc, kp, seed, first_id, id_stride, nullptr, (int64_t)0);
        HIPCHK(hipGetLastError());
    }
    return run_sweeps(h, GMRF_SOLVE_BACKWARD, kp);
}

gmrf_status gmrf_bt_sample(gmrf_handle* h, uint64_t seed, int64_t first_id, int64_t k, const double* mean,
                           const double* z, double* out, int64_t ld) {
    h = tw_route(h);
    if (!h || !out) return bad_shape("null pointer");
    if (!h->factored) { g_last_error = "sample before factor"; return GMRF_ERR_NO_FACTOR; }
    if (k <= 0 || ld < h->n) return bad_shape("bad k / ld");
    if (h->B > 1 && k > KP_CHUNK) return bad_shape("with a batch of problems k is limited to 128 per call");
    HIPCHK(hipSetDevice(h->device));
    if (tw_on(h)) return tw_sample(h, seed, first_id, k, mean, z, out, ld);
    const double* d_mean = nullptr;
    Staging args(h->mean_arena);
    args.in(mean, sizeof(double) * h->n * h->B, &d_mean);
    GCHK(args.commit(h->stream));
    const bool out_dev = is_device_ptr(out);
    const int64_t smp_bytes = cols_bytes(h->n, k * h->B, ld);
    GCHK(sweep_guarded(h, {{z, smp_bytes, out, smp_bytes}, {mean, h->n * h->B * (int64_t)sizeof(double), out, smp_bytes}},
                       [&]() -> gmrf_status {
        HIPCHK(hipEventRecord(h->ev0, h->stream));
        for (int64_t c0 = 0; c0 < k; c0 += KP_CHUNK) {
            const int kc = (int)std::min<int64_t>(KP_CHUNK, k - c0);
            GCHK(sample_chunk(h, seed, first_id + c0, kc, z ? z + c0 * ld : nullptr, ld, k));
            GCHK(cols_out(h, h->d_Y, kc, d_mean, out + c0 * ld, ld, out_dev));
            if (!out_dev) HIPCHK(hipStreamSynchronize(h->stream));
        }
        HIPCHK(hipEventRecord(h->ev1, h->stream));
        HIPCHK(hipStreamSynchronize(h->stream));
        return GMRF_OK;
    }));
    float ms = 0.f;
    (void)hipEventElapsedTime(&ms, h->ev0, h->ev1);
    h->stats.sample_ms = ms;
    if (h->profiling) prof_collect(h);
    return GMRF_OK;
}

static gmrf_status ensure_aux(gmrf_handle* h) {
    if (h->aux_distinct) return GMRF_OK;
    HIPCHK(hipStreamSynchronize(h->stream));
    if (h->aux) { (void)hipStreamSynchronize(h->aux); (void)hipStreamDestroy(h->aux); h->aux = nullptr; }
    const unsigned long long ticks = 100000ull;
    double one = 1e30;
    for (int r = 0; r < 2; ++r) one = std::min(one, spin_pair_ms(h->stream, nullptr, ticks));
    std::vector<hipStream_t> cand;
    for (int c = 0; c < 12 && !h->aux; ++c) {
        hipStream_t st = nullptr;
        HIPCHK(hipStreamCreateWithFlags(&st, hipStreamNonBlocking));
// ... 26 lines not shown
    }
    GCHK(ensure_aux(h));
    h->fork_next = 0;
    hipEvent_t ev_fork = nullptr, ev_join = nullptr;
    GCHK(fork_event(h, &ev_fork)); GCHK(fork_event(h, &ev_join));
    h->sweep_persist_launched = true;
    h->stats.sweep_persist = 1;
    h->stats.sweep_persist_launches += 3;
    HIPCHK(hipEventRecord(h->ev0, h->stream));
    HIPCHK(hipEventRecord(ev_fork, h->stream));
    HIPCHK(hipStreamWaitEvent(h->aux, ev_fork, 0));
    {
        const int64_t total = (int64_t)kp * h->n_pad;
        hipLaunchKernelGGL(fill_normals_panel, dim3((unsigned)((total + 255) / 256), 1), dim3(256), 0, h->aux, h->d_P2, h->n_pad,
                           (int)h->bs, (int)h->bsp, (int)k, kp, seed, first_id, k, nullptr, (int64_t)0);
        HIPCHK(hipGetLastError());
        GCHK(launch_sweep_persist(h, true, kp, h->d_P2, h->d_Y2, h->aux, h->d_T2));
        HIPCHK(hipEventRecord(ev_join, h->aux));
    }
    GCHK(launch_pack(h, b, h->n, 1, 1));
    GCHK(launch_sweep_persist(h, false, 1, h->d_P, h->d_Y));
    GCHK(launch_sweep_persist(h, true, 1, h->d_Y, h->d_P));
    GCHK(launch_unpack(h, h->d_P, mean, h->n, 1, nullptr));
    HIPCHK(hipStreamWaitEvent(h->stream, ev_join, 0));
    GCHK(launch_unpack(h, h->d_Y2, samples, ld, (int)k, mean));
    HIPCHK(hipEventRecord(h->ev1, h->stream));
    HIPCHK(hipStreamSynchronize(h->stream));
    return GMRF_OK;
}

static bool posterior_fused_ok(gmrf_handle* h, int64_t k, bool dev_all) {
    if (tw_on(h) || h->B <= 1 || !dev_all || h->no_fused_posterior || h->sweep_no_gemm || k <= 0 || k > KP_CHUNK) return false;
    const int kp = pad_k(k);
    if (kp % 64 != 0 || (int64_t)h->B * (h->bsp / 64) * (kp / 64) < 128) return false;
    if ((int64_t)(kp + 1) * h->n_pad * 8 >= ((int64_t)1 << 32)) return false;
    if (ensure_panels(h, kp + 1) != GMRF_OK) return false;
    if (!h->d_dout && hipMalloc(&h->d_dout, sizeof(GemmDirectOut)) != hipSuccess) { (void)hipGetLastError(); return false; }
    h->tail_probe = true; h->tail_refused = false;
    const gmrf_status st = sweep_launches(h, true, kp, h->d_P, h->d_Y, true, h->d_dout);
    h->tail_probe = false;
    return st == GMRF_OK && !h->tail_refused;
}

static gmrf_status posterior_fused(gmrf_handle* h, const double* b, uint64_t seed, int64_t first_id, int64_t k, double* mean,
                                   double* samples, int64_t ld) {
    const int kp = pad_k(k);
    GCHK(ensure_panels(h, kp + 1));
    HIPCHK(hipEventRecord(h->ev0, h->stream));
    const bool have_y = h->fy_for && b == h->fy_for;
    if (!have_y) {
        GCHK(launch_pack(h, b, h->n, 1, 1));
        GCHK(run_sweeps(h, GMRF_SOLVE_FORWARD, 1));
    }
    {
        const int64_t total = (int64_t)(kp + 1) * h->n_pad;
        hipLaunchKernelGGL(fill_normals_panel, dim3((unsigned)((total + 255) / 256), (unsigned)h->B), dim3(256), 0,
                           h->stream, h->d_P, h->n_pad, (int)h->bs, (int)h->bsp, (int)k, kp, seed, first_id, k,
                           have_y ? h->d_fy : h->d_Y, h->n_pad);
        HIPCHK(hipGetLastError());
    }
    hipLaunchKernelGGL(set_direct_out, dim3(1), dim3(1), 0, h->stream, h->d_dout, samples, mean, ld, k);
    HIPCHK(hipGetLastError());
    GCHK(run_sweeps(h, SWEEP_BACKWARD_TAIL, kp));
    HIPCHK(hipEventRecord(h->ev1, h->stream));
    HIPCHK(hipStreamSynchronize(h->stream));
    if (h->profiling) prof_collect(h);
    return GMRF_OK;
}

gmrf_status gmrf_bt_posterior(gmrf_handle* h, const double* b, uint64_t seed, int64_t first_id, int64_t k, double* mean,
                              double* samples, int64_t ld) {
    h = tw_route(h);
    if (!h || !b || !mean || !samples) return bad_shape("null pointer");
    if (!h->factored) { g_last_error = "posterior before factor"; return GMRF_ERR_NO_FACTOR; }
    if (k <= 0 || ld < h->n) return bad_shape("bad k / ld");
    HIPCHK(hipSetDevice(h->device));
    const bool dev_all = is_device_ptr(b) && is_device_ptr(mean) && is_device_ptr(samples);
    const int64_t vec_bytes = h->n * h->B * (int64_t)sizeof(double), smp_bytes = cols_bytes(h->n, k * h->B, ld);
    bool beside = false, fused = false;
    GCHK(sweep_guarded(h, {{b, vec_bytes, mean, vec_bytes}, {b, vec_bytes, samples, smp_bytes}, {mean, vec_bytes, samples, smp_bytes}},
                       [&]() -> gmrf_status {
        beside = !tw_on(h) && h->B == 1 && k <= KP_CHUNK && k >= 2 && dev_all && !h->profiling && sweep_persist_ok(h, 1) &&
                 sweep_persist_ok(h, pad_k(k));
        if (beside) return posterior_beside(h, b, seed, first_id, k, mean, samples, ld);
        fused = !h->sweep_persist_hold && posterior_fused_ok(h, k, dev_all);
        return fused ? posterior_fused(h, b, seed, first_id, k, mean, samples, ld) : GMRF_OK;
    }, [&]() -> gmrf_status {
        if (h->aux) HIPCHK(hipStreamSynchronize(h->aux));
        return GMRF_OK;
    }));
    if (!beside && !fused) {
        GCHK(gmrf_bt_solve(h, b, mean, 1, h->n, h->n, GMRF_SOLVE_FULL));
        return gmrf_bt_sample(h, seed, first_id, k, mean, nullptr, samples, ld);
    }
    float ms = 0.f;
    (void)hipEventElapsedTime(&ms, h->ev0, h->ev1);
    h->stats.solve_ms = ms;
    h->stats.sample_ms = 0.0;
    return GMRF_OK;
}

gmrf_status gmrf_bt_set_factor_rhs(gmrf_handle* h, const double* b) {
    if (!h) return bad_shape("null handle");
    if (b && !is_device_ptr(b)) return bad_shape("the factor's right-hand side must be device memory");
    h->frhs = b;
    h->fy_for = nullptr;
    return GMRF_OK;
}

gmrf_status gmrf_bt_normals(gmrf_handle* h, uint64_t seed, int64_t first_id, int64_t k, double* z, int64_t ld) {
    if (!h || !z) return bad_shape("null pointer");
    if (h->n <= 0) return bad_shape("no shape set");
    if (k <= 0 || ld < h->n) return bad_shape("bad k / ld");
    if (h->B > 1 && k > KP_CHUNK) return bad_shape("with a batch of problems k is limited to 128 per call");
    HIPCHK(hipSetDevice(h->device));
    const bool z_dev = is_device_ptr(z);
    for (int64_t c0 = 0; c0 < k; c0 += KP_CHUNK) {
        const int kc = (int)std::min<int64_t>(KP_CHUNK, k - c0);
        const int kp = pad_k(kc);
        GCHK(ensure_panels(h, kp));
        const int64_t total = (int64_t)kp * h->n_pad;
        hipLaunchKernelGGL(fill_normals_panel, dim3((unsigned)((total + 255) / 256), (unsigned)h->B), dim3(256), 0,
                           h->stream, h->d_P, h->n_pad, (int)h->bs, (int)h->bsp, kc, kp, seed, first_id + c0, k, nullptr, (int64_t)0);
        HIPCHK(hipGetLastError());
        GCHK(cols_out(h, h->d_P, kc, nullptr, z + c0 * ld, ld, z_dev));
        HIPCHK(hipStreamSynchronize(h->stream));
    }
    return GMRF_OK;
}

gmrf_status gmrf_bt_logdet(gmrf_handle* h, double* out) {
    h = tw_route(h);
    if (!h || !out) return bad_shape("null pointer");
    if (!h->factored) { g_last_error = "logdet before factor"; return GMRF_ERR_NO_FACTOR; }
    HIPCHK(hipSetDevice(h->device));
    if (tw_on(h)) return tw_logdet(h, out);
    if (h->keep_l && h->l_valid) {
        hipLaunchKernelGGL(logdet_blocks, dim3((unsigned)h->N, 1), dim3(256), 0, h->stream,
                           h->d_L + h->sel * stride_pL(h), blk_elems(h), h->bsp, (int)h->bs, h->d_logdet + h->sel * h->N,
                           (int64_t)0, (int64_t)0);
        HIPCHK(hipGetLastError());
    } else if (!h->logdet_valid) {
        g_last_error = "neither the L blocks nor the log-determinant parts of this factor are resident (adopted as raw buffers without L)";
        return GMRF_ERR_NO_FACTOR;
    }
    std::vector<double> part((size_t)h->N);
    HIPCHK(hipMemcpyAsync(part.data(), h->d_logdet + h->sel * h->N, sizeof(double) * h->N, hipMemcpyDeviceToHost, h->stream));
    HIPCHK(hipStreamSynchronize(h->stream));
    double s = 0.0;
    for (double v : part) s += v;
    *out = 2.0 * s;
    return GMRF_OK;
}

gmrf_status gmrf_csr_create(int32_t device, void* stream, int64_t n_rows, int64_t n_cols, const int64_t* rowptr,
                            const int64_t* colidx, const double* vals, int32_t index_base, int32_t values_f32,
                            gmrf_csr** out) {
    if (!out || !rowptr || !colidx || !vals || n_rows <= 0 || n_cols <= 0) return bad_shape("bad CSR arguments");
    std::unique_ptr<gmrf_csr, gmrf_status (*)(gmrf_csr*)> guard(new gmrf_csr(), gmrf_csr_destroy);
    gmrf_csr* m = guard.get();
    GCHK(m->open(device, stream, hipStreamNonBlocking, "gmrf_csr_create", false));
    const int64_t nnz = rowptr[n_rows] - index_base;
    if (nnz < 0 || rowptr[0] != index_base) return bad_shape("bad CSR row pointers");
    std::vector<int64_t> rp((size_t)n_rows + 1);
    for (int64_t i = 0; i <= n_rows; ++i) {
        rp[i] = rowptr[i] - index_base;
        if (i > 0 && rp[i] < rp[i - 1]) return bad_shape("CSR row pointers must be non-decreasing");
    }
    std::vector<int32_t> ci((size_t)nnz);
    for (int64_t p = 0; p < nnz; ++p) {
        const int64_t c = colidx[p] - index_base;
        if (c < 0 || c >= n_cols) return bad_shape("column index out of range");
        ci[p] = (int32_t)c;
    }
// ... 3223 lines not shown
gmrf_status gmrf_test_tile_timing(double* out, int32_t n) {
    if (!out || n < 18) return bad_shape("need 18 outputs");
    out[0] = g_tile_us;
    for (int i = 0; i < 17; ++i) out[1 + i] = (double)(g_tile_stamps[i] - g_tile_stamps[15]);
    if (n >= 24) for (int i = 0; i < 3; ++i) out[18 + i] = (double)(g_tile_stamps[20 + i] - g_tile_stamps[15]);
    if (n >= 30) for (int i = 0; i < 6; ++i) out[24 + i] = (double)(g_tile_stamps[24 + i] - g_tile_stamps[24]);
    if (n >= 62) for (int i = 0; i < 8; ++i) out[54 + i] = g_tile_stamps[56 + i] ? (double)(g_tile_stamps[56 + i] - g_tile_stamps[15]) : -1.0;
    if (n >= 54) for (int i = 0; i < 24; ++i) out[30 + i] = g_tile_stamps[32 + i] ? (double)(g_tile_stamps[32 + i] - g_tile_stamps[15]) : -1.0;
    return GMRF_OK;
}

gmrf_status gmrf_test_persist_stamps(double* out, int32_t n) {
    if (!out || n < 1 || n > 128) return bad_shape("1 .. 128 outputs");
    for (int i = 0; i < n; ++i)
        out[i] = g_persist_stamps[i] ? (g_persist_stamps[i] < 64 ? (double)g_persist_stamps[i] : (double)(g_persist_stamps[i] - g_persist_stamps[0])) : -1.0;
    return GMRF_OK;
}

gmrf_status gmrf_test_factor_fwd(gmrf_handle* h, int32_t* state, double* y_out) {
    if (!h || !state) return bad_shape("null pointer");
    HIPCHK(hipSetDevice(h->device));
    *state = (h->fy_for && h->factored && h->fy_for == h->frhs) ? 1 : 0;
    if (y_out && *state) {
        GCHK(cols_out(h, h->d_fy, 1, nullptr, y_out, h->n, false));
        HIPCHK(hipStreamSynchronize(h->stream));
    }
    return GMRF_OK;
}

gmrf_status gmrf_test_gn_route(gmrf_gn* g, int32_t* iterations, int32_t* fwd_iterations) {
    if (!g || !iterations || !fwd_iterations) return bad_shape("null pointer");
    *iterations = g->iterations; *fwd_iterations = g->fwd_iterations;
    return GMRF_OK;
}

gmrf_status gmrf_test_dc_route(gmrf_dc* g, int32_t* fwd_in_factor) {
    if (!g || !fwd_in_factor) return bad_shape("null pointer");
    *fwd_in_factor = g->fwd_in_factor;
    return GMRF_OK;
}

gmrf_status gmrf_test_bic_route(gmrf_bic* g, int32_t* fwd_in_factor) {
    if (!g || !fwd_in_factor) return bad_shape("null pointer");
    *fwd_in_factor = g->fwd_in_factor;
    return GMRF_OK;
}

gmrf_status gmrf_test_var_groups(gmrf_handle* h, int32_t* group_size, int32_t* groups) {
    if (!h || !group_size || !groups) return bad_shape("null pointer");
    *group_size = h->var_group; *groups = h->var_groups;
    return GMRF_OK;
}

gmrf_status gmrf_test_persist_aborts(gmrf_handle* h, int32_t* n) {
    if (!h || !n) return bad_shape("null argument");
    *n = h->persist_aborts;
    return GMRF_OK;
}

gmrf_status gmrf_test_persist_budget(int32_t cus, int32_t n, const int32_t* demands, int32_t* granted) {
    if (n < 0 || (n > 0 && (!demands || !granted))) return bad_shape("null argument");
    std::map<const void*, int> claims;
    for (int i = 0; i < n; ++i) granted[i] = persist_budget_claim(claims, (const void*)(demands + i), demands[i], cus, 0) ? 1 : 0;
    return GMRF_OK;
}

gmrf_status gmrf_test_potrf_block(int32_t device, int64_t bs, double* S, double* Linv, int32_t* info) {
    if (bs % 64 || next_pow2(bs / 64) != bs / 64) return bad_shape("bs must be 64 * 2^p");
    gmrf_handle* h = nullptr;
    GCHK(gmrf_bt_create(device, nullptr, &h));
    h->N = 1; h->n = bs; h->bs = bs; h->bsp = bs; h->n_pad = bs; h->B = 1;
    gmrf_status s = set_layout_dense(h);
    if (s == GMRF_OK) s = alloc_factor(h);
    unsigned long long* dst = nullptr;
    if (s == GMRF_OK && hipMalloc(&dst, 128 * sizeof(unsigned long long)) == hipSuccess) {
        (void)hipMemset(dst, 0, 128 * sizeof(unsigned long long));
        h->dbg_stamps = dst;
    }
    if (s == GMRF_OK) {
        hipError_t e = hipMemcpyAsync(h->d_S, S, sizeof(double) * bs * bs, hipMemcpyHostToDevice, h->stream);
        persist_plan(h);
        if (e == hipSuccess) s = potrf_block(h, h->d_S, h->d_L, h->d_Linv, h->d_T, 1);
        if (s == GMRF_OK) {
            int hi = 0;
            (void)hipMemcpyAsync(&hi, h->d_info, sizeof(int), hipMemcpyDeviceToHost, h->stream);
            (void)hipMemcpyAsync(S, h->d_L, sizeof(double) * bs * bs, hipMemcpyDeviceToHost, h->stream);
            (void)hipMemcpyAsync(Linv, h->d_Linv, sizeof(double) * bs * bs, hipMemcpyDeviceToHost, h->stream);
            if (hipStreamSynchronize(h->stream) != hipSuccess) s = GMRF_ERR_HIP;
            if (info) *info = hi;
            if (dst) (void)hipMemcpy(g_tile_stamps + 24, dst, 6 * sizeof(unsigned long long), hipMemcpyDeviceToHost);
            if (dst) (void)hipMemcpy(g_persist_stamps, dst, 128 * sizeof(unsigned long long), hipMemcpyDeviceToHost);
        }
    }
    if (dst) (void)hipFree(dst);
    gmrf_bt_destroy(h);
    return s;
}

gmrf_status gmrf_test_potrf_route(int32_t device, int64_t bs, int32_t batch, int32_t eager_bits, int64_t cmin, int32_t keep_l,
                                  double* S, double* L, double* Linv, int32_t* info, int32_t* route) {
    if (!S || !L || !Linv || !info || !route) return bad_shape("null pointer");
    if (bs < 64 || bs % 64 || next_pow2(bs / 64) != bs / 64) return bad_shape("bs must be 64 * 2^p");
    if (batch < 1) return bad_shape("batch must be >= 1");
    if (cmin < 0 || cmin >= bs || cmin % 64) return bad_shape("cmin must be a multiple of 64 in [0, bs)");
    gmrf_handle* h = nullptr;
    GCHK(gmrf_bt_create(device, nullptr, &h));
// ... 166 lines not shown
```

diffeqgmrfs.jl_amd/csrc/misc_kernels.hpp:

```cpp
#pragma once
#include <hip/hip_runtime.h>
#include <stdint.h>

namespace gmrf {

__global__ void scatter_block(const uint64_t* __restrict__ keys, const double* __restrict__ vals,
                              int64_t first, int64_t count, double* __restrict__ dst, int64_t ld,
                              int64_t pvals, int64_t pdst, int add) {
    const int64_t i = (int64_t)blockIdx.x * blockDim.x + threadIdx.x;
    if (i >= count) return;
    const uint64_t key = keys[first + i];
    const int64_t r = (int64_t)(key >> 32), c = (int64_t)(key & 0xffffffffu);
    double* d = dst + (int64_t)blockIdx.y * pdst + r * ld + c;
    const double v = vals[(int64_t)blockIdx.y * pvals + first + i];
    *d = add ? *d + v : v;
}

__global__ void zero_rows(double* __restrict__ dst, int64_t count, int64_t pdst) {
    const int64_t i = ((int64_t)blockIdx.x * blockDim.x + threadIdx.x) * 2;
    if (i < count) *reinterpret_cast<v2d*>(dst + (int64_t)blockIdx.y * pdst + i) = (v2d){0.0, 0.0};
}

__global__ void pad_identity(double* __restrict__ dst, int64_t ld, int bs, int bsp, int64_t pdst) {
    const int i = bs + blockIdx.x * blockDim.x + threadIdx.x;
// ... 52 lines not shown
    double v = 0.0;
    if (r < k && off < bs) v = src[((int64_t)blockIdx.y * k + r) * ld + blk * bs + off];
    P[(int64_t)blockIdx.y * total + idx] = v;
}

__global__ void unpack_panel(const double* __restrict__ P, int64_t n_pad, double* __restrict__ dst,
                             int64_t ld, int bs, int bsp, int64_t n, int k, int kp,
                             const double* __restrict__ mean) {
    const int64_t idx = (int64_t)blockIdx.x * blockDim.x + threadIdx.x;
    if (idx >= n * (int64_t)k) return;
    const int64_t r = idx / n, j = idx % n;
    const int64_t blk = j / bs, off = j % bs;
    double v = P[(int64_t)blockIdx.y * kp * n_pad + r * n_pad + blk * bsp + off];
    if (mean) v += mean[(int64_t)blockIdx.y * n + j];
    dst[((int64_t)blockIdx.y * k + r) * ld + j] = v;
}

__device__ __host__ inline void philox4x32_10(uint32_t c[4], uint32_t k0, uint32_t k1) {
    for (int i = 0; i < 10; ++i) {
        const uint64_t p0 = (uint64_t)0xD2511F53u * c[0];
        const uint64_t p1 = (uint64_t)0xCD9E8D57u * c[2];
        const uint32_t n0 = (uint32_t)(p1 >> 32) ^ c[1] ^ k0;
        const uint32_t n1 = (uint32_t)p1;
        const uint32_t n2 = (uint32_t)(p0 >> 32) ^ c[3] ^ k1;
        const uint32_t n3 = (uint32_t)p0;
        c[0] = n0; c[1] = n1; c[2] = n2; c[3] = n3;
        k0 += 0x9E3779B9u; k1 += 0xBB67AE85u;
    }
}

__device__ __host__ inline double philox_normal(uint64_t seed, uint64_t dof, uint64_t sample) {
    uint32_t c[4] = {(uint32_t)dof, (uint32_t)(dof >> 32), (uint32_t)sample, (uint32_t)(sample >> 32)};
    philox4x32_10(c, (uint32_t)seed, (uint32_t)(seed >> 32));
    const uint64_t a = ((uint64_t)c[1] << 32) | c[0];
    const uint64_t b = ((uint64_t)c[3] << 32) | c[2];
    const double u1 = ((double)(a >> 11) + 0.5) * (1.0 / 9007199254740992.0);
    const double u2 = ((double)(b >> 11) + 0.5) * (1.0 / 9007199254740992.0);
    return sqrt(-2.0 * log(u1)) * cos(6.283185307179586476925 * u2);
}

__global__ void fill_normals_panel(double* __restrict__ P, int64_t n_pad, int bs, int bsp,
                                   int k, int kp, uint64_t seed, int64_t first_id, int64_t id_stride,
                                   const double* __restrict__ yrow, int64_t ystride) {
    const int64_t idx = (int64_t)blockIdx.x * blockDim.x + threadIdx.x;
    const int rows = kp + (yrow ? 1 : 0);
    if (idx >= (int64_t)rows * n_pad) return;
    const int64_t r = idx / n_pad, j = idx % n_pad;
    const int64_t blk = j / bsp, off = j % bsp;
    double v = 0.0;
    if (r == kp) v = yrow[(int64_t)blockIdx.y * ystride + j];
    else if (r < k && off < bs)
        v = philox_normal(seed, (uint64_t)(blk * bs + off), (uint64_t)(first_id + (int64_t)blockIdx.y * id_stride + r));
    P[(int64_t)blockIdx.y * rows * n_pad + idx] = v;
}

struct BxtArgs {
    const int* rowptr;
    const uint64_t* keys;
    const double* vals;
    int64_t n_entries;
    const double* X;
    double* C;
    int64_t ld, ldc, pX, pC;
    const int* kst;
    int cm, rm, bsp;
    int cw;
};

template <int KM>
__global__ __launch_bounds__(256) void spmm_bxt(BxtArgs a) {
    const int ncc = (a.bsp - a.cm) / a.cw, nrc = (a.rm + 255) / 256;
    const int nprob = (int)gridDim.x / (ncc * nrc);
    int cc, rc, prob;
    {
        const int groups = (nprob % 8 == 0) ? 8 : 1;
        const int xg = (int)blockIdx.x % groups, q = (int)blockIdx.x / groups;
        rc = q % nrc;
        cc = (q / nrc) % ncc;
        prob = xg + groups * (q / (nrc * ncc));
    }
    const int r = rc * 256 + (int)threadIdx.x;
    const int c0 = a.cm + cc * a.cw;
    const double* __restrict__ X = a.X + (int64_t)prob * a.pX;
    double* __restrict__ C = a.C + (int64_t)prob * a.pC;
    const double* __restrict__ vals = a.vals + (int64_t)prob * a.n_entries;
    int k0 = 0, len = 0;
    if (r < a.rm) { k0 = a.rowptr[r]; len = a.rowptr[r + 1] - k0; }
    int jt[KM];
    double vt[KM];
#pragma unroll
    for (int t = 0; t < KM; ++t) {
        const bool ok = t < len;
        jt[t] = ok ? (int)(a.keys[k0 + t] & 0xffffffffu) : 0;
        vt[t] = ok ? vals[k0 + t] : 0.0;
    }
    int lm = len;
#pragma unroll
    for (int off = 32; off > 0; off >>= 1) lm = max(lm, __shfl_xor(lm, off));
    lm = __builtin_amdgcn_readfirstlane(lm);
    __shared__ double ls[256 * 17];
    const int tid = (int)threadIdx.x;
    const int wr = tid >> 4, wc = tid & 15;
    const int rbase = rc * 256;
    const int cfirst = a.cm + (a.kst ? a.kst[rbase >> 6] : 0);
    for (int c = c0; c < c0 + a.cw; c += 16) {
        if (c + 16 <= cfirst) continue;
// ... 959 lines not shown
```

diffeqgmrfs.jl_amd/csrc/potrf_step.hpp:

```cpp
#pragma once
#include <hip/hip_runtime.h>
#include <stdint.h>

#include "gemm_f64.hpp"

#ifndef GMRF_TILE_EXACT_DIV
#define GMRF_TILE_EXACT_DIV 0
#endif

namespace gmrf {

#ifndef GMRF_PANEL_FLAT_LDS
#define GMRF_PANEL_FLAT_LDS 0
#endif
#ifndef GMRF_TLD
#define GMRF_TLD 66
#endif
constexpr int TLD = GMRF_TLD;
constexpr int TILE_ELEMS = 64 * TLD;
__device__ __forceinline__ double bcast_lane(double v, int src) {
    const int lo = __builtin_amdgcn_readlane(__double2loint(v), src);
    const int hi = __builtin_amdgcn_readlane(__double2hiint(v), src);
    return __hiloint2double(hi, lo);
}

__device__ __forceinline__ double rsqrt_nr(double p) {
    const double y = __builtin_amdgcn_rsq(p);
    const double e = fma(-p * y, y, 1.0);
    const double c = fma(0.375, e, 0.5);
    return fma(y * e, c, y);
}

__device__ __forceinline__ v4d mm16_nt(const double* a, int lda, const double* b, int ldb, v4d acc,
                                       bool negate, int li, int lq) {
#pragma unroll
    for (int ks = 0; ks < 4; ++ks) {
        double av = a[li * lda + 4 * ks + lq];
        const double bv = b[li * ldb + 4 * ks + lq];
        if (negate) av = -av;
        acc = __builtin_amdgcn_mfma_f64_16x16x4f64(av, bv, acc, 0, 0, 0);
    }
    return acc;
}

__device__ __forceinline__ v4d mm16_nn(const double* a, int lda, const double* b, int ldb, v4d acc,
                                       bool negate, int li, int lq) {
#pragma unroll
    for (int ks = 0; ks < 4; ++ks) {
        double av = a[li * lda + 4 * ks + lq];
        const double bv = b[(4 * ks + lq) * ldb + li];
        if (negate) av = -av;
        acc = __builtin_amdgcn_mfma_f64_16x16x4f64(av, bv, acc, 0, 0, 0);
    }
    return acc;
}

__device__ __forceinline__ v4d load_d16(const double* p, int ld, int li, int lq) {
// ... 787 lines not shown
    __syncthreads();
    tile_potrf_inv(Ts, Xs, Wk, rinvs, tid, bad, side);
    tile_s2g(Ts, sa.L + o0 * ld + o0, ld, tid);
    tile_s2g(Xs, sa.X + o0 * ld + o0, ld, tid);
    v4d lr[4];
#pragma unroll
    for (int Jb = 0; Jb < 4; ++Jb) lr[Jb] = zero;
#pragma unroll
    for (int kg = 0; kg < 8; ++kg) {
        const int k = 8 * kg + 2 * lq;
        const v2d av = *reinterpret_cast<const v2d*>(As + (16 * wave + li) * TLD + k);
#pragma unroll
        for (int Jb = kg / 2; Jb < 4; ++Jb) {
            const v2d xv = *reinterpret_cast<const v2d*>(Xs + (16 * Jb + li) * TLD + k);
            lr[Jb] = __builtin_amdgcn_mfma_f64_16x16x4f64(av.x, xv.x, lr[Jb], 0, 0, 0);
            lr[Jb] = __builtin_amdgcn_mfma_f64_16x16x4f64(av.y, xv.y, lr[Jb], 0, 0, 0);
        }
    }
    __syncthreads();
#pragma unroll
    for (int Jb = 0; Jb < 4; ++Jb) store_d16(As + (16 * wave) * TLD + 16 * Jb, TLD, lr[Jb], li, lq);
    __syncthreads();
    tile_s2g(As, sa.L + o1 * ld + o0, ld, tid);
    v4d pacc[4], wv[4];
#pragma unroll
    for (int Jb = 0; Jb < 4; ++Jb) { pacc[Jb] = zero; wv[Jb] = zero; }
    strip_syrk_and_w_w(wave, As + (16 * wave + li) * TLD, As, Xs, pacc, wv, li, lq);
    __syncthreads();
#pragma unroll
    for (int Jb = 0; Jb < 4; ++Jb) {
        store_d16(As + (16 * wave) * TLD + 16 * Jb, TLD, wv[Jb], li, lq);
        if (Jb <= wave) {
#pragma unroll
            for (int q = 0; q < 4; ++q) Ts[(16 * wave + lq + 4 * q) * TLD + 16 * Jb + li] = cpre[Jb][q] - pacc[Jb][q];
        }
    }
    __syncthreads();
    NoSide none;
    tile_potrf_inv(Ts, Xs, Wk, rinvs, tid, bad, none);
    if (bad && tid == 0) atomicCAS(sa.info, 0, sa.blk);
    tile_s2g(Ts, sa.L + o1 * ld + o1, ld, tid);
    tile_s2g(Xs, sa.X + o1 * ld + o1, ld, tid);
    v4d xr[4];
#pragma unroll
    for (int Jb = 0; Jb < 4; ++Jb) xr[Jb] = zero;
    strip_tri_nn_w(wave, Xs + (16 * wave + li) * TLD, As, xr, li, lq);
#pragma unroll
    for (int Jb = 0; Jb < 4; ++Jb)
#pragma unroll
        for (int q = 0; q < 4; ++q) sa.X[(o1 + 16 * wave + lq + 4 * q) * ld + o0 + 16 * Jb + li] = -xr[Jb][q];
}
constexpr size_t POTRF_DIAG128_LDS = (3 * TILE_ELEMS + WK_ELEMS + 64) * sizeof(double);

__global__ __launch_bounds__(256, 1) void potrf_diag128_slim(StepArgs sa) {
    sa.S += (int64_t)blockIdx.y * sa.pS;
    sa.L += (int64_t)blockIdx.y * sa.pL;
    sa.X += (int64_t)blockIdx.y * sa.pX;
    sa.blk += (int)blockIdx.y * sa.blk_per_problem;
    extern __shared__ __attribute__((aligned(16))) double smem[];
    double* Ts = smem;
    double* Xs = Ts + TILE_ELEMS;
    double* Wk = Xs + TILE_ELEMS;
    double* rinvs = Wk + WK_ELEMS;
    const int tid = threadIdx.x;
    const int lane = tid & 63, wave = __builtin_amdgcn_readfirstlane(tid >> 6);
    const int li = lane & 15, lq = lane >> 4;
    const int64_t ld = sa.ld;
    const int64_t o0 = (int64_t)sa.j * 64, o1 = o0 + 64;
    const v4d zero = (v4d){0.0, 0.0, 0.0, 0.0};
    v4d cpre[4];
#pragma unroll
    for (int Jb = 0; Jb < 4; ++Jb)
#pragma unroll
        for (int q = 0; q < 4; ++q)
            cpre[Jb][q] = (Jb <= wave) ? sa.S[(o1 + 16 * wave + lq + 4 * q) * ld + o1 + 16 * Jb + li] : 0.0;
    v2d s10[8];
#pragma unroll
    for (int kg = 0; kg < 8; ++kg)
        s10[kg] = *reinterpret_cast<const v2d*>(sa.S + (o1 + 16 * wave + li) * ld + o0 + 8 * kg + 2 * lq);
    bool bad = false;
    tile_g2s(sa.S + o0 * ld + o0, ld, Ts, tid);
    NoSide none;
    __syncthreads();
    tile_potrf_inv(Ts, Xs, Wk, rinvs, tid, bad, none);
    tile_s2g(Ts, sa.L + o0 * ld + o0, ld, tid);
    tile_s2g(Xs, sa.X + o0 * ld + o0, ld, tid);
    v4d lr[4];
#pragma unroll
    for (int Jb = 0; Jb < 4; ++Jb) lr[Jb] = zero;
#pragma unroll
    for (int kg = 0; kg < 8; ++kg) {
        const int k = 8 * kg + 2 * lq;
#pragma unroll
        for (int Jb = kg / 2; Jb < 4; ++Jb) {
            const v2d xv = *reinterpret_cast<const v2d*>(Xs + (16 * Jb + li) * TLD + k);
            lr[Jb] = __builtin_amdgcn_mfma_f64_16x16x4f64(s10[kg].x, xv.x, lr[Jb], 0, 0, 0);
            lr[Jb] = __builtin_amdgcn_mfma_f64_16x16x4f64(s10[kg].y, xv.y, lr[Jb], 0, 0, 0);
        }
    }
    __syncthreads();
#pragma unroll
    for (int Jb = 0; Jb < 4; ++Jb) store_d16(Ts + (16 * wave) * TLD + 16 * Jb, TLD, lr[Jb], li, lq);
    __syncthreads();
    tile_s2g(Ts, sa.L + o1 * ld + o0, ld, tid);
    v4d pacc[4], wv[4];
#pragma unroll
    for (int Jb = 0; Jb < 4; ++Jb) { pacc[Jb] = zero; wv[Jb] = zero; }
    strip_syrk_and_w_w(wave, Ts + (16 * wave + li) * TLD, Ts, Xs, pacc, wv, li, lq);
    __syncthreads();
#pragma unroll
    for (int Jb = 0; Jb < 4; ++Jb) {
// ... 52 lines not shown
```

diffeqgmrfs.jl_amd/posterior.py:

```python
from __future__ import annotations

from typing import List, Optional, Tuple

import numpy as np


def shard_range(total: int, world: int, rank: int) -> Tuple[int, int]:
    base, rem = divmod(total, world)
    first = rank * base + min(rank, rem)
    return first, base + (1 if rank < rem else 0)


def block_groups(n_blocks: int, group: int) -> List[Tuple[int, int]]:
    return [(i, min(n_blocks, i + group)) for i in range(0, n_blocks, group)]


class HipEngine:

    def __init__(self, pkg, workload, device_index: int = 0, batch: int = 1, values=None, rhs=None,
                 keep_l: bool = True, transport: str = "torch", comm=None):
        import torch
        self.torch = torch
        self.pkg = pkg
        self.w = workload
# ... 158 lines not shown
        if dist.get_backend() == "nccl":
            self._pending.append((dist.all_gather_into_tensor(allb, own, async_op=True), i0, i1, allb))
        else:
            b = self.share_batch
            allb[self.rank * b:(self.rank + 1) * b].copy_(own)
            hs = [dist.broadcast(allb[r * b:(r + 1) * b], src=r, async_op=True) for r in range(self.world)]
            for h in hs[:-1]:
                self._pending.append((h, None, None, None))
            self._pending.append((hs[-1], i0, i1, allb))
        self.bytes_moved += (allb.numel() - own.numel()) * 8

    def share_finish(self, is_root: bool = True):
        if self.transport == "cabi":
            self.comm.wait(self.F_all)
            return
        for hnd, i0, i1, allb in self._pending:
            hnd.wait()
            if allb is not None:
                self.F_all.unpack_blocks_async(i0, i1, allb)
        self._pending = []

    def mean(self):
        return self.F_all.solve_batch(self.rhs)[:, 0, :]

    def sample(self, k: int, mean, seed: int, first_id: int, keep: bool = True):
        if k <= 128:
            return self.F_all.sample_batch(k, mean=mean, seed=seed, first_id=first_id, like=self.rhs)
        outs = []
        for c0 in range(0, k, 128):
            kc = min(128, k - c0)
            x = self.F_all.sample_batch(kc, mean=mean, seed=seed, first_id=first_id + c0 * self.batch, like=self.rhs)
            outs = outs + [x] if keep else [x]
        return self.torch.cat(outs, dim=1) if keep else outs[0]


class ShardedPosterior:

    def __init__(self, engine, dist=None, rank: int = 0, world: int = 1, k_samples: int = 64,
                 seed: int = 0x5EED, group: int = 8, replicate_factor: bool = False, force_shared: bool = False,
                 keep_samples: bool = True, timing: bool = False, share: str = "broadcast"):
        self.e, self.dist, self.rank, self.world = engine, dist, rank, world
        self.k, self.seed, self.group = k_samples, seed, group
        self.replicate = replicate_factor or (world == 1 and not force_shared)
        self.groups = block_groups(engine.w.n_blocks, group)
        self.keep_samples = keep_samples
        self.share = share
        if share not in ("broadcast", "allgather"):
            raise ValueError(share)
        if share == "allgather":
            self.replicate = False
        self.timing = timing and hasattr(engine, "torch")
        self._ev = None

    def prepare(self):
        self.e.prepare(is_root=(self.rank == 0), shared_storage=not self.replicate, dist=self.dist)
        if self.dist is not None and self.world > 1:
            self.dist.barrier()

    def _mark(self, i: int):
        if self.timing:
            self._ev[i].record(self.e.torch.cuda.current_stream(self.e.dev))

    def _factor_and_share(self):
        if self.timing and self._ev is None:
            self._ev = [self.e.torch.cuda.Event(enable_timing=True) for _ in range(4)]
        self._mark(0)
        if self.replicate:
            self.e.factor()
            self._mark(1); self._mark(2)
            return
        if self.share == "allgather":
            for gi, (i0, i1) in enumerate(self.groups):
                self.e.factor_range_async(i0, i1, first=(gi == 0))
                self.e.share_range(self.dist, i0, i1, True)
            self._mark(1)
            self.e.factor_end()
            self.e.share_finish(True)
            self._mark(2)
            self.e.adopt_commit()
            return
        root = self.rank == 0
        for gi, (i0, i1) in enumerate(self.groups):
            if root:
                self.e.factor_range_async(i0, i1, first=(gi == 0))
            self.e.share_range(self.dist, i0, i1, root)
        self._mark(1)
        self.e.share_finish(root)
        self._mark(2)
        if root:
            self.e.factor_end()
        else:
            self.e.adopt_commit()

    def step(self, step_index: int = 0):
        self._factor_and_share()
        nb = getattr(self.e, "batch", 1)
        first = (step_index * self.world + self.rank) * self.k * nb
        if self.replicate and type(self.e) is HipEngine:
            mu, X = self.e.posterior(self.k, self.seed, first, keep=self.keep_samples)
        else:
            mu = self.e.mean()
            X = self.e.sample(self.k, mu, self.seed, first) if self.keep_samples else self.e.sample(self.k, mu, self.seed, first, keep=False)
        self._mark(3)
        return mu, X

    def phase_ms(self):
        if not self.timing or self._ev is None:
            return None
        e = self._ev
        return {"factor_ms": e[0].elapsed_time(e[1]), "transfer_wait_ms": e[1].elapsed_time(e[2]),
                "mean_and_samples_ms": e[2].elapsed_time(e[3])}

    def solves_per_step(self) -> int:
        nb = getattr(self.e, "batch", 1)
        if self.replicate:
            return self.world * nb * (1 + self.k)
        return nb * (1 + self.k * self.world)
```

include/gmrf_hip.h:

```cpp
#ifndef GMRF_HIP_H
#define GMRF_HIP_H

#include <stdint.h>

#ifdef __cplusplus
extern "C" {
#endif

typedef int32_t gmrf_status;

enum {
    GMRF_OK = 0,
    GMRF_ERR_NOT_SPD = -1,
    GMRF_ERR_BAD_SHAPE = -2,
    GMRF_ERR_BAND = -3,
    GMRF_ERR_HIP = -4,
    GMRF_ERR_NO_FACTOR = -5,
    GMRF_ERR_NO_DEVICE = -6,
    GMRF_ERR_ALLOC = -7,
    GMRF_ERR_RCCL = -8
};

enum { GMRF_SOLVE_FULL = 0, GMRF_SOLVE_FORWARD = 1, GMRF_SOLVE_BACKWARD = 2 };
enum { GMRF_VAR_EXACT = 0, GMRF_VAR_RBMC = 1, GMRF_VAR_MC = 2 };
enum { GMRF_BLOCK_L = 0, GMRF_BLOCK_C = 1, GMRF_BLOCK_LINV = 2 };

typedef struct gmrf_handle gmrf_handle;
typedef struct gmrf_csr gmrf_csr;
typedef struct gmrf_comm gmrf_comm;

typedef struct {
    int64_t nnz;
    const int64_t* ptr;
    const int64_t* idx;
    const double* val;
} gmrf_sparse_block;

typedef struct {
    double factor_ms;
    double solve_ms;
    double sample_ms;
    double factor_flops;
    double sweep_bytes;
    double sweep_ms;
    int64_t n, n_blocks, block_size, block_size_padded;
    int64_t factor_bytes;
#define GMRF_KERNEL_CLASSES 24
    double kernel_ms[GMRF_KERNEL_CLASSES];
    double kernel_work[GMRF_KERNEL_CLASSES];
    int64_t kernel_launches[GMRF_KERNEL_CLASSES];
    double sweep_bytes_streamed;
    int32_t persist_route;
    int32_t persist_aborts;
    int32_t persist_cus;
    int32_t persist_refused;
    int32_t sweep_persist;
    int32_t sweep_persist_launches;
} gmrf_stats;


gmrf_status gmrf_bt_create(int32_t device, void* stream, gmrf_handle** out);
gmrf_status gmrf_bt_destroy(gmrf_handle* h);
const char* gmrf_last_error(void);
int32_t gmrf_version(void);

gmrf_status gmrf_bt_factor_csc(gmrf_handle* h, int64_t n, int64_t n_blocks,
                               const int64_t* colptr, const int64_t* rowval,
                               const double* nzval, int32_t index_base, int32_t* info);

gmrf_status gmrf_bt_factor_blocks(gmrf_handle* h, int64_t n, int64_t n_blocks,
                                  const gmrf_sparse_block* diag,
                                  const gmrf_sparse_block* lower,
                                  int32_t index_base, int32_t compressed_by_column,
                                  int32_t* info);

gmrf_status gmrf_bt_refactor_values(gmrf_handle* h, const double* nzval, int32_t* info);

gmrf_status gmrf_bt_solve(gmrf_handle* h, const double* b, double* y, int64_t k,
                          int64_t ldb, int64_t ldy, int32_t mode);

gmrf_status gmrf_bt_sample(gmrf_handle* h, uint64_t seed, int64_t first_id, int64_t k,
                           const double* mean, const double* z, double* out, int64_t ld);

gmrf_status gmrf_bt_posterior(gmrf_handle* h, const double* b, uint64_t seed, int64_t first_id, int64_t k,
                              double* mean, double* samples, int64_t ld);

gmrf_status gmrf_bt_set_factor_rhs(gmrf_handle* h, const double* b);

gmrf_status gmrf_bt_normals(gmrf_handle* h, uint64_t seed, int64_t first_id, int64_t k,
                            double* z, int64_t ld);

gmrf_status gmrf_bt_marginal_var(gmrf_handle* h, int32_t method, int64_t k, uint64_t seed,
                                 const gmrf_csr* Q, double* var_out);

gmrf_status gmrf_bt_marginal_var_batch(gmrf_handle* h, int32_t method, int64_t k, uint64_t seed,
                                       const gmrf_csr* Q, const double* q_vals, double* var_out);

gmrf_status gmrf_bt_selinv(gmrf_handle* h, const gmrf_csr* S, double* vals_out);

gmrf_status gmrf_bt_trace_inv(gmrf_handle* h, const gmrf_csr* S, const double* dvals, int64_t m, double* out);

gmrf_status gmrf_bt_var_accumulate(gmrf_handle* h, int32_t method, int64_t first_id,
                                   int64_t k, uint64_t seed, const gmrf_csr* Q,
                                   double* acc);

gmrf_status gmrf_bt_logdet(gmrf_handle* h, double* out);

gmrf_status gmrf_bt_get_block(gmrf_handle* h, int32_t kind, int64_t i, double* out,
                              int64_t ld);

gmrf_status gmrf_bt_export_size(gmrf_handle* h, int64_t* bytes);
gmrf_status gmrf_bt_export_factor(gmrf_handle* h, void* host_buf, int64_t bytes);
gmrf_status gmrf_bt_import_factor(gmrf_handle* h, const void* host_buf, int64_t bytes);

gmrf_status gmrf_bt_factor_buffer(gmrf_handle* h, int32_t kind, void** dev_ptr,
                                  int64_t* bytes);
gmrf_status gmrf_bt_block_range(gmrf_handle* h, int32_t kind, int64_t i0, int64_t i1,
                                int64_t* first_elem, int64_t* n_elems, int64_t* problem_stride);
gmrf_status gmrf_bt_set_keep_l(gmrf_handle* h, int32_t keep);
gmrf_status gmrf_bt_get_layout(gmrf_handle* h, int64_t* out, int64_t cap, int64_t* count);

gmrf_status gmrf_bt_packed_size(gmrf_handle* h, int64_t i0, int64_t i1, int64_t* elems_per_problem);
gmrf_status gmrf_bt_pack_blocks_async(gmrf_handle* h, int64_t i0, int64_t i1, double* dev_buf);
gmrf_status gmrf_bt_unpack_blocks_async(gmrf_handle* h, int64_t i0, int64_t i1, const double* dev_buf);

gmrf_status gmrf_bt_storage_bytes(int64_t n, int64_t n_blocks, int64_t batch, int64_t* bytes_L,
                                  int64_t* bytes_C, int64_t* bytes_Linv);
gmrf_status gmrf_bt_set_storage(gmrf_handle* h, int64_t n, int64_t n_blocks, int64_t batch,
                                void* dev_L, void* dev_C, void* dev_Linv);

gmrf_status gmrf_bt_adopt_layout(gmrf_handle* h, int64_t n, int64_t n_blocks,
                                 const int64_t* layout, int64_t count);
gmrf_status gmrf_bt_adopt_shape(gmrf_handle* h, int64_t n, int64_t n_blocks);
gmrf_status gmrf_bt_adopt_commit(gmrf_handle* h, int32_t l_blocks_valid);

gmrf_status gmrf_comm_unique_id(void* id128);
gmrf_status gmrf_comm_create(int32_t device, int32_t rank, int32_t world, const void* id128,
                             gmrf_comm** out);
gmrf_status gmrf_comm_destroy(gmrf_comm* c);
gmrf_status gmrf_comm_bcast_host(gmrf_comm* c, void* host_buf, int64_t bytes, int32_t root);
// ... 124 lines not shown
gmrf_status gmrf_elliptic_p1_tangent(gmrf_elliptic_p1* e, const double* w, double* vals_out, double* f_out);
gmrf_status gmrf_elliptic_p1_tangent_batch(gmrf_elliptic_p1* e, int64_t batch, const double* w, double* vals_out, double* f_out);
gmrf_status gmrf_elliptic_p1_load(gmrf_elliptic_p1* e, int64_t batch, const double* src_q, double* b_out);
gmrf_status gmrf_elliptic_p2_create(int32_t device, void* stream, int64_t nx, int64_t ny, gmrf_elliptic_p1** out);
gmrf_status gmrf_gn_create_elliptic(gmrf_handle* h, gmrf_assembler* as, gmrf_elliptic_p1* e, gmrf_gn** out);

gmrf_status gmrf_darcy_p1_assemble_batch(gmrf_darcy_p1* d, int64_t batch, const double* coeff_tables, int64_t ng, double beta,
                                         double* vals_out, double* f_out);
typedef struct gmrf_dc gmrf_dc;
gmrf_status gmrf_dc_create(gmrf_handle* h, gmrf_assembler* as, gmrf_darcy_p1* d, gmrf_dc** out);
gmrf_status gmrf_dc_destroy(gmrf_dc* g);
gmrf_status gmrf_dc_run(gmrf_dc* g, const double* coeff_tables, int64_t ng, double beta, const double* q_nzval, int64_t q_stride,
                        const double* q_mu, double q_eps, int64_t k_samples, uint64_t sample_seed, int32_t var_method, int64_t k_var,
                        uint64_t var_seed, double* mean_out, double* samples_out, double* std_out, double* std_norm_out,
                        int32_t* info);

typedef struct gmrf_swe_p1 gmrf_swe_p1;
gmrf_status gmrf_shallow_water_p1_create(int32_t device, void* stream, int64_t nx, int64_t ny, gmrf_swe_p1** out);
gmrf_status gmrf_shallow_water_p1_destroy(gmrf_swe_p1* w);
gmrf_status gmrf_shallow_water_p1_pattern(const gmrf_swe_p1* w, int32_t which, int64_t* nnz_out, int64_t* rowptr, int64_t* colidx,
                                          int32_t index_base);
gmrf_status gmrf_shallow_water_p1_qpoints(const gmrf_swe_p1* w, double* xy);
gmrf_status gmrf_shallow_water_p1_assemble(gmrf_swe_p1* w, const double* H_q, double k, double f, double g, const uint8_t* prescribed,
                                           double* K_vals, double* M_lumped, double* S_vals);
gmrf_status gmrf_shallow_water_p1_operators(gmrf_swe_p1* w, const double* K_vals, const double* M_lumped, const double* S_vals,
                                            const uint8_t* prescribed, double kappa_matern, double tau, double dt, double* G_vals,
                                            double* J_vals, double* M_tilde, double* beta);

gmrf_status gmrf_test_gemm(int32_t device, int64_t M, int64_t N, int64_t K, int32_t transA,
                           int32_t transB, int32_t tri_flags, int32_t lower_only,
                           double alpha, const double* A, int64_t lda, const double* B,
                           int64_t ldb, double beta, double* C, int64_t ldc);
gmrf_status gmrf_test_gemm_pair(int32_t device, int32_t batch, int32_t grouped, const int64_t* desc, const double* ab,
                                const double* A0, const double* B0, double* C0, const double* A1, const double* B1, double* C1);
gmrf_status gmrf_test_gemm_desc(int32_t device, int32_t route, const int64_t* desc, const double* abt,
                                const double* A, int64_t nA, const double* B, int64_t nB, double* C, int64_t nC,
                                const double* D, int64_t nD, const double* tA, int64_t ntA, double* tC, int64_t ntC,
                                const double* tD, int64_t ntD, const int32_t* kb_m, int64_t n_kb_m, const int32_t* kb_n,
                                int64_t n_kb_n, const int32_t* ke_n, int64_t n_ke_n, double* samples, int64_t n_samples,
                                double* mean, int64_t n_mean, int32_t* family);
gmrf_status gmrf_test_gemm_rate(int32_t device, int64_t M, int64_t N, int64_t K, int32_t transB,
                                int32_t tri_flags, int32_t lower_only, int32_t batch,
                                int32_t big, int32_t reps, double* ms_per_launch);
gmrf_status gmrf_test_gemm_shapes(gmrf_handle* h, double* rows, int64_t cap_rows, int64_t* n_rows);
gmrf_status gmrf_test_potrf_tile(int32_t device, double* tile64 ,
                                 double* inv64, int32_t* info);
gmrf_status gmrf_test_tile_timing(double* out, int32_t n);
gmrf_status gmrf_test_potrf_block(int32_t device, int64_t bs, double* S ,
                                  double* Linv, int32_t* info);
gmrf_status gmrf_test_potrf_route(int32_t device, int64_t bs, int32_t batch, int32_t eager_bits, int64_t cmin, int32_t keep_l,
                                  double* S, double* L, double* Linv, int32_t* info, int32_t* route);
gmrf_status gmrf_test_persist_stamps(double* out, int32_t n);
gmrf_status gmrf_test_persist_aborts(gmrf_handle* h, int32_t* n);
gmrf_status gmrf_test_factor_fwd(gmrf_handle* h, int32_t* state, double* y_out);
gmrf_status gmrf_test_gn_route(gmrf_gn* g, int32_t* iterations, int32_t* fwd_iterations);
gmrf_status gmrf_test_dc_route(gmrf_dc* g, int32_t* fwd_in_factor);
gmrf_status gmrf_test_bic_route(gmrf_bic* g, int32_t* fwd_in_factor);
gmrf_status gmrf_test_var_groups(gmrf_handle* h, int32_t* group_size, int32_t* groups);
gmrf_status gmrf_test_persist_budget(int32_t cus, int32_t n, const int32_t* demands, int32_t* granted);
gmrf_status gmrf_test_mfma_f64_rate(int32_t device, double* tflops);
gmrf_status gmrf_test_clock_probe_start(int32_t device, int32_t n, int32_t sleeps, void** probe);
gmrf_status gmrf_test_clock_probe_finish(void* probe, double* ghz, double* t_ms);
gmrf_status gmrf_test_hbm_rate(int32_t device, int64_t bytes, double* gbps);
gmrf_status gmrf_test_microbench(int32_t device, double* out, int32_t n);
gmrf_status gmrf_test_symbolic_csc(int64_t n, int64_t n_blocks, const int64_t* colptr, const int64_t* rowval,
                                   int32_t index_base, int64_t* out8);

#ifdef __cplusplus
}
#endif
#endif
```

Baseline: 54160 solves/s.

## Generate posterior normal draws inside the factorization's diag128 potrf launches

Adds extra 'rider' workgroups to the potrf_diag128_slim kernel. During the Cholesky factor, these fill slices of the sample panel with Philox normals, using CUs that would otherwise idle during the latency-bound diagonal step. The posterior then only copies in the RHS row instead of launching a separate fill_normals_panel, when the draws registered for the factor match the request. This adds bookkeeping to invalidate the pre-drawn panel, graph-recapture keys, and a changed launch grid for the diagonal kernel (problem index moves to x). Rider work may slow the critical-path potrf if it contends for resources.

```diff
diff --git a/diffeqgmrfs.jl_amd/_cabi.py b/diffeqgmrfs.jl_amd/_cabi.py
--- a/diffeqgmrfs.jl_amd/_cabi.py
+++ b/diffeqgmrfs.jl_amd/_cabi.py
@@ -17,7 +17,7 @@
 EXPORTS = [
     "gmrf_bt_create", "gmrf_bt_destroy", "gmrf_last_error", "gmrf_version",
     "gmrf_bt_factor_csc", "gmrf_bt_factor_blocks", "gmrf_bt_refactor_values",
-    "gmrf_bt_solve", "gmrf_bt_sample", "gmrf_bt_posterior", "gmrf_bt_set_factor_rhs", "gmrf_bt_normals", "gmrf_bt_marginal_var",
+    "gmrf_bt_solve", "gmrf_bt_sample", "gmrf_bt_posterior", "gmrf_bt_set_factor_rhs", "gmrf_bt_set_factor_draws", "gmrf_bt_normals", "gmrf_bt_marginal_var",
     "gmrf_bt_var_accumulate", "gmrf_bt_logdet", "gmrf_bt_get_block", "gmrf_bt_factor_buffer",
     "gmrf_bt_adopt_shape", "gmrf_bt_adopt_commit", "gmrf_bt_adopt_layout", "gmrf_bt_get_layout", "gmrf_bt_block_range",
     "gmrf_bt_set_keep_l", "gmrf_bt_storage_bytes", "gmrf_bt_set_storage", "gmrf_bt_factor_begin_csc",
@@ -40,7 +40,7 @@
     "gmrf_darcy_p1_assemble_batch", "gmrf_dc_create", "gmrf_dc_destroy", "gmrf_dc_run",
     "gmrf_burgers_prior_create", "gmrf_burgers_line_prior_create", "gmrf_burgers_prior_destroy", "gmrf_burgers_prior_pattern", "gmrf_burgers_prior_values_batch",
     "gmrf_bic_create", "gmrf_bic_destroy", "gmrf_bic_run", "gmrf_field_errors_batch",
-    "gmrf_test_gemm", "gmrf_test_gemm_desc", "gmrf_test_gemm_pair", "gmrf_test_gemm_rate", "gmrf_test_gemm_shapes", "gmrf_test_potrf_tile", "gmrf_test_potrf_block", "gmrf_test_potrf_route", "gmrf_test_tile_timing", "gmrf_test_persist_stamps", "gmrf_test_persist_aborts", "gmrf_test_factor_fwd", "gmrf_test_gn_route", "gmrf_test_dc_route", "gmrf_test_bic_route", "gmrf_test_var_groups", "gmrf_test_persist_budget", "gmrf_test_clock_probe_start", "gmrf_test_clock_probe_finish",
+    "gmrf_test_gemm", "gmrf_test_gemm_desc", "gmrf_test_gemm_pair", "gmrf_test_gemm_rate", "gmrf_test_gemm_shapes", "gmrf_test_potrf_tile", "gmrf_test_potrf_block", "gmrf_test_potrf_route", "gmrf_test_tile_timing", "gmrf_test_persist_stamps", "gmrf_test_persist_aborts", "gmrf_test_draw_slice", "gmrf_test_drawn_panel", "gmrf_test_factor_fwd", "gmrf_test_gn_route", "gmrf_test_dc_route", "gmrf_test_bic_route", "gmrf_test_var_groups", "gmrf_test_persist_budget", "gmrf_test_clock_probe_start", "gmrf_test_clock_probe_finish",
     "gmrf_test_mfma_f64_rate", "gmrf_test_hbm_rate", "gmrf_test_microbench", "gmrf_test_symbolic_csc",
 ]
 
@@ -58,7 +58,7 @@
         ("kernel_ms", C.c_double * 24), ("kernel_work", C.c_double * 24), ("kernel_launches", C.c_int64 * 24),
         ("sweep_bytes_streamed", C.c_double),
         ("persist_route", C.c_int32), ("persist_aborts", C.c_int32), ("persist_cus", C.c_int32), ("persist_refused", C.c_int32),
-        ("sweep_persist", C.c_int32), ("sweep_persist_launches", C.c_int32),
+        ("sweep_persist", C.c_int32), ("sweep_persist_launches", C.c_int32), ("posterior_draws_in_factor", C.c_int32),
     ]
 
 
@@ -102,6 +102,7 @@
         "gmrf_bt_sample": [vp, u64, i64, i64, vp, vp, vp, i64],
         "gmrf_bt_posterior": [vp, vp, u64, i64, i64, vp, vp, i64],
         "gmrf_bt_set_factor_rhs": [vp, vp],
+        "gmrf_bt_set_factor_draws": [vp, i64, u64, i64],
         "gmrf_bt_normals": [vp, u64, i64, i64, vp, i64],
         "gmrf_bt_marginal_var": [vp, i32, i64, u64, vp, vp],
         "gmrf_bt_var_accumulate": [vp, i32, i64, i64, u64, vp, vp],
@@ -218,6 +219,8 @@
         "gmrf_test_tile_timing": [vp, i32],
         "gmrf_test_persist_stamps": [vp, i32],
         "gmrf_test_persist_aborts": [vp, vp],
+        "gmrf_test_draw_slice": [u64, u64, u64, P(u64)],
+        "gmrf_test_drawn_panel": [vp, P(i64), vp],
         "gmrf_test_factor_fwd": [vp, vp, vp],
         "gmrf_test_gn_route": [vp, P(i32), P(i32)],
         "gmrf_test_dc_route": [vp, vp],
diff --git a/diffeqgmrfs.jl_amd/api.py b/diffeqgmrfs.jl_amd/api.py
--- a/diffeqgmrfs.jl_amd/api.py
+++ b/diffeqgmrfs.jl_amd/api.py
@@ -1077,6 +1077,9 @@
         self._factor_rhs = b
         _cabi.check(self._lib.gmrf_bt_set_factor_rhs(self._h, _cabi.ptr(b)))
 
+    def set_factor_draws(self, k: int, seed: int = 0x5EED, first_id: int = 0):
+        _cabi.check(self._lib.gmrf_bt_set_factor_draws(self._h, int(k), int(seed), int(first_id)))
+
     def marginal_var(self, method: str = "exact", k: int = 50, seed: int = 0x5EED, Q: Optional[CsrMatrix] = None,
                      q_values=None, out=None):
         m = {"exact": _cabi.VAR_EXACT, "rbmc": _cabi.VAR_RBMC, "mc": _cabi.VAR_MC}[method]
diff --git a/diffeqgmrfs.jl_amd/csrc/gmrf_hip.hip b/diffeqgmrfs.jl_amd/csrc/gmrf_hip.hip
--- a/diffeqgmrfs.jl_amd/csrc/gmrf_hip.hip
+++ b/diffeqgmrfs.jl_amd/csrc/gmrf_hip.hip
@@ -214,6 +214,15 @@
     double* d_fy = nullptr;
     int64_t fy_elems = 0;
     const double* factor_graph_rhs = nullptr;
+    int64_t draw_k = 0, draw_first = 0;
+    uint64_t draw_seed = 0;
+    int64_t drawn_k = 0, drawn_first = 0;
+    uint64_t drawn_seed = 0;
+    bool draws_run = false;
+    bool no_factor_draws = false;
+    DrawRecord* d_draw_rec = nullptr;
+    const double* factor_graph_draw_P = nullptr;
+    int factor_graph_draw_kp = 0;
     unsigned long long* dbg_stamps = nullptr;
     bool fork_graph = false;
     bool no_staircase = false;
@@ -631,6 +640,7 @@
 
 static gmrf_status ensure_panels(gmrf_handle* h, int64_t kp) {
     if (kp <= h->kp_cap && h->d_P) return GMRF_OK;
+    h->drawn_k = 0;
     for (auto& kv : h->sweep_graphs) (void)hipGraphExecDestroy(kv.second);
     h->sweep_graphs.clear();
     free_dev(h->d_P); free_dev(h->d_Y); free_dev(h->d_Tp);
@@ -1077,6 +1087,20 @@
     return GMRF_OK;
 }
 
+static int pad_k(int64_t k);
+static bool diag128_fat() {
+    static const bool fat = [] { const char* e = getenv("GMRF_DIAG128_FAT"); return e && atoi(e) != 0; }();
+    return fat;
+}
+static bool persist_panels_on(const gmrf_handle* h) {
+    static const bool no_small = [] { const char* e = getenv("GMRF_PERSIST_PANELS"); return e && atoi(e) == 0; }();
+    return !no_small && !h->no_persist_panels && persist_fits(h, 4, 0, 4, 2);
+}
+static int draw_riders() {
+    static const int r = [] { const char* e = getenv("GMRF_DRAW_RIDERS"); const int v = e ? atoi(e) : 1; return v < 1 ? 1 : (v > 16 ? 16 : v); }();
+    return r;
+}
+
 static gmrf_status potrf_block(gmrf_handle* h, double* S, double* L, double* X, double* T, int blk_id, double* fy = nullptr) {
     const int bsp = (int)h->bsp;
     const int64_t ld = bsp;
@@ -1140,14 +1164,29 @@
             sa.j = j;
             ProfScope ps(h, 16, (2.0 * t3 / 3.0 + 4.0 * 2.0 * t3 * 0.625) * nb);
             static const size_t lds_pad = [] { const char* e = getenv("GMRF_DIAG128_LDS_PAD_KB"); return (size_t)(e ? atoi(e) : 0) * 1024; }();
-            static const bool fat = [] { const char* e = getenv("GMRF_DIAG128_FAT"); return e && atoi(e) != 0; }();
-            if (fat) hipLaunchKernelGGL(potrf_diag128, dim3(1, (unsigned)h->B), dim3(256), POTRF_DIAG128_LDS + lds_pad, h->stream, sa);
-            else hipLaunchKernelGGL(potrf_diag128_slim, dim3(1, (unsigned)h->B), dim3(256), POTRF_DIAG128_SLIM_LDS + lds_pad, h->stream, sa);
+            if (diag128_fat()) {
+                if (h->draws_run) return bad_shape("internal: draws planned off potrf_diag128_slim");
+                hipLaunchKernelGGL(potrf_diag128, dim3(1, (unsigned)h->B), dim3(256), POTRF_DIAG128_LDS + lds_pad, h->stream, sa);
+            } else {
+                RiderArgs ra{};
+                if (h->draws_run) {
+                    ra.rec = h->d_draw_rec; ra.P = h->d_P; ra.n_pad = h->n_pad; ra.bs = (int)h->bs;
+                    ra.lg_bsp = 0;
+                    while ((1 << ra.lg_bsp) < bsp) ++ra.lg_bsp;
+                    const uint64_t s = (uint64_t)(((blk_id - 1) * (nt / 4) + j / 4) * 2 + ((j % 4) ? 1 : 0)), S = (uint64_t)h->N * (uint64_t)(nt / 2);
+                    ra.kp = pad_k(h->draw_k);
+                    const uint64_t T = (uint64_t)ra.kp * (uint64_t)h->n_pad;
+                    ra.lo = (uint32_t)draw_slice(T, S, s); ra.hi = (uint32_t)draw_slice(T, S, s + 1);
+                    ra.riders = draw_riders();
+                }
+                hipLaunchKernelGGL(potrf_diag128_slim, dim3((unsigned)h->B, 1 + (unsigned)ra.riders), dim3(256), POTRF_DIAG128_SLIM_LDS + lds_pad,
+                                   h->stream, sa, ra);
+            }
             HIPCHK(hipGetLastError());
             return GMRF_OK;
         };
-        static const bool no_small = [] { const char* e = getenv("GMRF_PERSIST_PANELS"); return e && atoi(e) == 0; }();
-        const bool persist_panels = !no_small && !h->no_persist_panels && persist_fits(h, 4, 0, 4, 2);
+        const bool persist_panels = persist_panels_on(h);
+        if (persist_panels && h->draws_run) return bad_shape("internal: draws planned off potrf_diag128_slim");
         for (int j = 0; j < nt; j += 4) {
             const int64_t oa = (int64_t)j * 64, ob = oa + 128, oc = oa + 256;
             if (persist_panels) {
@@ -1481,10 +1520,30 @@
     return GMRF_OK;
 }
 
+static bool posterior_fused_ok(gmrf_handle* h, int64_t k, bool dev_all);
+
+static gmrf_status factor_draws_ok(gmrf_handle* h, bool* ok) {
+    *ok = false;
+    if (h->draw_k <= 0 || h->no_factor_draws || h->B <= 1 || tw_on(h) || h->tw_blk >= 0 || h->fork_graph) return GMRF_OK;
+    if (potrf_route(h) != ROUTE_PANELS256 || h->bsp % 256 != 0 || diag128_fat() || persist_panels_on(h)) return GMRF_OK;
+    if (!posterior_fused_ok(h, h->draw_k, true)) return GMRF_OK;
+    if (!h->d_draw_rec) HIPCHK(hipMalloc(&h->d_draw_rec, sizeof(DrawRecord)));
+    *ok = true;
+    return GMRF_OK;
+}
+
 static gmrf_status run_factor(gmrf_handle* h, int64_t i0, int64_t i1) {
+    if (h->draws_run) {
+        hipLaunchKernelGGL(set_draw_record, dim3(1), dim3(1), 0, h->stream, h->d_draw_rec, h->draw_seed, h->draw_first, (int)h->draw_k,
+                           pad_k(h->draw_k));
+        HIPCHK(hipGetLastError());
+    }
     if (h->eager || h->profiling) { h->stats.persist_route = 0; return factor_blocks_range(h, i0, i1); }
     const double* grhs = h->fwd_run ? h->frhs : nullptr;
-    if (!h->factor_graph || h->factor_graph_i0 != i0 || h->factor_graph_i1 != i1 || h->factor_graph_rhs != grhs) {
+    const double* gdraw = h->draws_run ? h->d_P : nullptr;
+    const int gkp = h->draws_run ? pad_k(h->draw_k) : 0;
+    if (!h->factor_graph || h->factor_graph_i0 != i0 || h->factor_graph_i1 != i1 || h->factor_graph_rhs != grhs ||
+        h->factor_graph_draw_P != gdraw || h->factor_graph_draw_kp != gkp) {
         std::lock_guard<std::mutex> capture_lock(g_capture_mu);
         if (h->factor_graph) { (void)hipGraphExecDestroy(h->factor_graph); h->factor_graph = nullptr; }
         hipGraph_t graph = nullptr;
@@ -1499,7 +1558,7 @@
         HIPCHK(e);
         HIPCHK(hipGraphInstantiate(&h->factor_graph, graph, nullptr, nullptr, 0));
         (void)hipGraphDestroy(graph);
-        h->factor_graph_i0 = i0; h->factor_graph_i1 = i1; h->factor_graph_rhs = grhs;
+        h->factor_graph_i0 = i0; h->factor_graph_i1 = i1; h->factor_graph_rhs = grhs; h->factor_graph_draw_P = gdraw; h->factor_graph_draw_kp = gkp;
     }
     h->xsplit = planned_xsplit(h);
     h->stats.persist_route = h->factor_graph_route;
@@ -1558,17 +1617,20 @@
     GCHK(load_values(h, nzval));
     HIPCHK(hipMemsetAsync(h->d_info, 0, 4 * sizeof(int), h->stream));
     h->info_checked = 0; h->persist_launched = false;
-    h->fy_for = nullptr;
-    bool fwd = false;
+    h->fy_for = nullptr; h->drawn_k = 0;
+    bool fwd = false, draws = false;
     GCHK(factor_fwd_ok(h, &fwd));
+    GCHK(factor_draws_ok(h, &draws));
     h->fwd_run = fwd;
+    h->draws_run = draws;
     gmrf_status s = run_factor(h, 0, h->N);
     if (s == GMRF_OK) {
         (void)hipEventRecord(h->ev1, h->stream);
         s = factor_finish(h, info);
     }
-    h->fwd_run = false;
+    h->fwd_run = false; h->draws_run = false;
     if (s == GMRF_OK && fwd) h->fy_for = h->frhs;
+    if (s == GMRF_OK && draws) { h->drawn_k = h->draw_k; h->drawn_seed = h->draw_seed; h->drawn_first = h->draw_first; }
     float ms = 0.f;
     (void)hipEventElapsedTime(&ms, h->ev0, h->ev1);
     h->stats.factor_ms = ms;
@@ -1838,6 +1900,7 @@
 
 constexpr int SWEEP_BACKWARD_YP = 3, SWEEP_BACKWARD_TAIL = 4;
 static gmrf_status run_sweeps(gmrf_handle* h, int mode, int kp) {
+    h->drawn_k = 0;
     auto body = [&]() -> gmrf_status {
         if (mode == GMRF_SOLVE_FORWARD) return sweep_launches(h, false, kp, h->d_P, h->d_Y);
         if (mode == SWEEP_BACKWARD_TAIL) return sweep_launches(h, true, kp, h->d_P, h->d_Y, true, h->d_dout);
@@ -1877,6 +1940,7 @@
 static int pad_k(int64_t k) { return k == 1 ? 1 : (int)((k + 15) / 16 * 16); }
 
 static gmrf_status launch_pack(gmrf_handle* h, const double* d_src, int64_t ld, int k, int kp) {
+    h->drawn_k = 0;
     const int64_t total = (int64_t)kp * h->n_pad;
     hipLaunchKernelGGL(pack_panel, dim3((unsigned)((total + 255) / 256), (unsigned)h->B), dim3(256), 0, h->stream, d_src, ld,
                        h->d_P, h->n_pad, (int)h->bs, (int)h->bsp, (int)h->N, k, kp);
@@ -1978,7 +2042,7 @@
     free_dev(h->d_S); free_dev(h->d_B); free_dev(h->d_T); free_dev(h->d_W);
     free_dev(h->d_sweep_flags); free_dev(h->d_Tsw); free_dev(h->d_P2); free_dev(h->d_Y2); free_dev(h->d_T2);
     if (h->h_sweep_abort) { (void)hipHostFree(h->h_sweep_abort); h->h_sweep_abort = nullptr; }
-    free_dev(h->d_dout); free_dev(h->d_info); free_dev(h->d_logdet); free_dev(h->d_pflags); free_dev(h->d_kbx); free_dev(h->d_V);
+    free_dev(h->d_dout); free_dev(h->d_draw_rec); free_dev(h->d_info); free_dev(h->d_logdet); free_dev(h->d_pflags); free_dev(h->d_kbx); free_dev(h->d_V);
     free_dev(h->d_P); free_dev(h->d_Y); free_dev(h->d_Tp);
     free_dev(h->d_stage); h->mean_arena.release(); free_dev(h->d_acc);
     free_dev(h->d_ft); free_dev(h->d_fy);
@@ -2042,7 +2106,8 @@
     h->no_fused_posterior = (eager & 262144) != 0;
     h->no_factor_fwd = (eager & 524288) != 0;
     if (((eager & 1048576) != 0) != h->no_grouped_gemm) { destroy_graphs(h); h->no_grouped_gemm = (eager & 1048576) != 0; }
-    if (eager != h->eager_bits) h->fy_for = nullptr;
+    if (((eager & 2097152) != 0) != h->no_factor_draws) { destroy_graphs(h); h->no_factor_draws = (eager & 2097152) != 0; }
+    if (eager != h->eager_bits) { h->fy_for = nullptr; h->drawn_k = 0; }
     h->eager = (eager & 1) != 0;
     h->eager_bits = eager;
     if (h->tw)
@@ -2108,7 +2173,7 @@
     GCHK(load_values(h, nzval));
     HIPCHK(hipMemsetAsync(h->d_info, 0, 4 * sizeof(int), h->stream));
     h->info_checked = 0; h->persist_launched = false; h->stats.persist_route = 0;
-    h->factored = false; h->fy_for = nullptr;
+    h->factored = false; h->fy_for = nullptr; h->drawn_k = 0;
     return GMRF_OK;
 }
 
@@ -2290,7 +2355,7 @@
     if (seen < 0) { g_last_error = "the packed ranges of this factor carry different (or no) representation tags"; return GMRF_ERR_BAD_SHAPE; }
     const int xs = seen > 0 ? seen - 1 : h->adopt_xsplit;
     if (xs < 0 || xs >= h->bsp || xs % 64) { g_last_error = "bad representation tag in the packed image"; return GMRF_ERR_BAD_SHAPE; }
-    h->factored = true; h->fy_for = nullptr;
+    h->factored = true; h->fy_for = nullptr; h->drawn_k = 0;
     h->xsplit = xs;
     h->l_valid = l_blocks_valid != 0 && h->keep_l;
     bool all = !h->got_block.empty();
@@ -2530,7 +2595,7 @@
     for (int64_t i = 0; i + 1 < N; ++i) GCHK(put(in + i * be, h->d_C + h->sel * stride_pC(h) + i * c_blk(h), false));
     in += (N - 1) * be;
     for (int64_t i = 0; i < N; ++i) GCHK(put(in + i * be, h->d_Linv + h->sel * stride_pX(h) + i * blk_elems(h), true));
-    h->factored = true; h->fy_for = nullptr; h->l_valid = true;
+    h->factored = true; h->fy_for = nullptr; h->drawn_k = 0; h->l_valid = true;
     persist_plan(h);
     h->xsplit = 0;
     return GMRF_OK;
@@ -2799,6 +2864,7 @@
         GCHK(launch_pack(h, d_z, ldd, kc, kp));
     } else {
         const int64_t total = (int64_t)kp * h->n_pad;
+        h->drawn_k = 0;
         hipLaunchKernelGGL(fill_normals_panel, dim3((unsigned)((total + 255) / 256), (unsigned)h->B), dim3(256), 0,
                            h->stream, h->d_P, h->n_pad, (int)h->bs, (int)h->bsp, kc, kp, seed, first_id, id_stride, nullptr, (int64_t)0);
         HIPCHK(hipGetLastError());
@@ -2931,7 +2997,13 @@
         GCHK(launch_pack(h, b, h->n, 1, 1));
         GCHK(run_sweeps(h, GMRF_SOLVE_FORWARD, 1));
     }
-    {
+    const bool drawn = h->drawn_k > 0 && h->drawn_k == k && h->drawn_seed == seed && h->drawn_first == first_id;
+    h->stats.posterior_draws_in_factor = drawn ? 1 : 0;
+    if (drawn) {
+        hipLaunchKernelGGL(panel_y_row, dim3((unsigned)((h->n_pad + 255) / 256), (unsigned)h->B), dim3(256), 0, h->stream, h->d_P, h->n_pad,
+                           kp, have_y ? h->d_fy : h->d_Y, h->n_pad);
+        HIPCHK(hipGetLastError());
+    } else {
         const int64_t total = (int64_t)(kp + 1) * h->n_pad;
         hipLaunchKernelGGL(fill_normals_panel, dim3((unsigned)((total + 255) / 256), (unsigned)h->B), dim3(256), 0,
                            h->stream, h->d_P, h->n_pad, (int)h->bs, (int)h->bsp, (int)k, kp, seed, first_id, k,
@@ -2955,6 +3027,7 @@
     if (k <= 0 || ld < h->n) return bad_shape("bad k / ld");
     HIPCHK(hipSetDevice(h->device));
     const bool dev_all = is_device_ptr(b) && is_device_ptr(mean) && is_device_ptr(samples);
+    h->stats.posterior_draws_in_factor = 0;
     const int64_t vec_bytes = h->n * h->B * (int64_t)sizeof(double), smp_bytes = cols_bytes(h->n, k * h->B, ld);
     bool beside = false, fused = false;
     GCHK(sweep_guarded(h, {{b, vec_bytes, mean, vec_bytes}, {b, vec_bytes, samples, smp_bytes}, {mean, vec_bytes, samples, smp_bytes}},
@@ -2987,6 +3060,13 @@
     return GMRF_OK;
 }
 
+gmrf_status gmrf_bt_set_factor_draws(gmrf_handle* h, int64_t k, uint64_t seed, int64_t first_id) {
+    if (!h) return bad_shape("null handle");
+    if (k < 0) return bad_shape("bad k");
+    h->draw_k = k; h->draw_seed = seed; h->draw_first = first_id;
+    return GMRF_OK;
+}
+
 gmrf_status gmrf_bt_normals(gmrf_handle* h, uint64_t seed, int64_t first_id, int64_t k, double* z, int64_t ld) {
     if (!h || !z) return bad_shape("null pointer");
     if (h->n <= 0) return bad_shape("no shape set");
@@ -2999,6 +3079,7 @@
         const int kp = pad_k(kc);
         GCHK(ensure_panels(h, kp));
         const int64_t total = (int64_t)kp * h->n_pad;
+        h->drawn_k = 0;
         hipLaunchKernelGGL(fill_normals_panel, dim3((unsigned)((total + 255) / 256), (unsigned)h->B), dim3(256), 0,
                            h->stream, h->d_P, h->n_pad, (int)h->bs, (int)h->bsp, kc, kp, seed, first_id + c0, k, nullptr, (int64_t)0);
         HIPCHK(hipGetLastError());
@@ -6328,6 +6409,22 @@
     return GMRF_OK;
 }
 
+gmrf_status gmrf_test_draw_slice(uint64_t T, uint64_t S, uint64_t s, uint64_t* first) {
+    if (!first || S == 0 || s > S) return bad_shape("bad S / s");
+    *first = draw_slice(T, S, s);
+    return GMRF_OK;
+}
+
+gmrf_status gmrf_test_drawn_panel(gmrf_handle* h, int64_t* k, double* out) {
+    if (!h || !k) return bad_shape("null pointer");
+    HIPCHK(hipSetDevice(h->device));
+    HIPCHK(hipStreamSynchronize(h->stream));
+    *k = h->drawn_k;
+    if (out && h->drawn_k > 0)
+        HIPCHK(hipMemcpy(out, h->d_P, sizeof(double) * (size_t)(h->B * (pad_k(h->drawn_k) + 1) * h->n_pad), hipMemcpyDeviceToHost));
+    return GMRF_OK;
+}
+
 gmrf_status gmrf_test_persist_aborts(gmrf_handle* h, int32_t* n) {
     if (!h || !n) return bad_shape("null argument");
     *n = h->persist_aborts;
diff --git a/diffeqgmrfs.jl_amd/csrc/misc_kernels.hpp b/diffeqgmrfs.jl_amd/csrc/misc_kernels.hpp
--- a/diffeqgmrfs.jl_amd/csrc/misc_kernels.hpp
+++ b/diffeqgmrfs.jl_amd/csrc/misc_kernels.hpp
@@ -128,6 +128,57 @@
     else if (r < k && off < bs)
         v = philox_normal(seed, (uint64_t)(blk * bs + off), (uint64_t)(first_id + (int64_t)blockIdx.y * id_stride + r));
     P[(int64_t)blockIdx.y * rows * n_pad + idx] = v;
+}
+
+
+__host__ __device__ inline uint64_t draw_slice(uint64_t T, uint64_t S, uint64_t s) { return s * T / S; }
+
+struct DrawRecord {
+    uint64_t seed;
+    int64_t first_id;
+    int k, kp;
+};
+
+__global__ void set_draw_record(DrawRecord* r, uint64_t seed, int64_t first_id, int k, int kp) {
+    r->seed = seed; r->first_id = first_id; r->k = k; r->kp = kp;
+}
+
+struct RiderArgs {
+    const DrawRecord* rec;
+    double* P;
+    int64_t n_pad;
+    int bs, lg_bsp;
+    uint32_t lo, hi;
+    int kp;
+    int riders;
+};
+
+__device__ inline void draw_rider(const RiderArgs& ra, int rider, int p, int tid) {
+    const DrawRecord rec = *ra.rec;
+    if (rec.kp != ra.kp) return;
+    const uint32_t n_pad = (uint32_t)ra.n_pad;
+    const uint32_t lo = ra.lo, hi = ra.hi;
+    const uint32_t step = (uint32_t)ra.riders * 256u;
+    uint32_t idx = lo + (uint32_t)rider * 256u + (uint32_t)tid;
+    if (idx >= hi) return;
+    uint32_t r = idx / n_pad, j = idx - r * n_pad;
+    double* __restrict__ dst = ra.P + (int64_t)p * ((int64_t)(rec.kp + 1) * ra.n_pad);
+    const uint32_t mask = (1u << ra.lg_bsp) - 1u;
+    const uint64_t id0 = (uint64_t)(rec.first_id + (int64_t)p * rec.k);
+    for (; idx < hi; idx += step) {
+        const uint32_t blk = j >> ra.lg_bsp, off = j & mask;
+        double v = 0.0;
+        if ((int)r < rec.k && (int)off < ra.bs) v = philox_normal(rec.seed, (uint64_t)blk * (uint64_t)ra.bs + off, id0 + r);
+        dst[idx] = v;
+        j += step;
+        while (j >= n_pad) { j -= n_pad; ++r; }
+    }
+}
+
+__global__ void panel_y_row(double* __restrict__ P, int64_t n_pad, int kp, const double* __restrict__ yrow, int64_t ystride) {
+    const int64_t j = (int64_t)blockIdx.x * blockDim.x + threadIdx.x;
+    if (j >= n_pad) return;
+    P[((int64_t)blockIdx.y * (kp + 1) + kp) * n_pad + j] = yrow[(int64_t)blockIdx.y * ystride + j];
 }
 
 struct BxtArgs {
diff --git a/diffeqgmrfs.jl_amd/csrc/potrf_step.hpp b/diffeqgmrfs.jl_amd/csrc/potrf_step.hpp
--- a/diffeqgmrfs.jl_amd/csrc/potrf_step.hpp
+++ b/diffeqgmrfs.jl_amd/csrc/potrf_step.hpp
@@ -3,6 +3,7 @@
 #include <stdint.h>
 
 #include "gemm_f64.hpp"
+#include "misc_kernels.hpp"
 
 #ifndef GMRF_TILE_EXACT_DIV
 #define GMRF_TILE_EXACT_DIV 0
@@ -896,11 +897,13 @@
 }
 constexpr size_t POTRF_DIAG128_LDS = (3 * TILE_ELEMS + WK_ELEMS + 64) * sizeof(double);
 
-__global__ __launch_bounds__(256, 1) void potrf_diag128_slim(StepArgs sa) {
-    sa.S += (int64_t)blockIdx.y * sa.pS;
-    sa.L += (int64_t)blockIdx.y * sa.pL;
-    sa.X += (int64_t)blockIdx.y * sa.pX;
-    sa.blk += (int)blockIdx.y * sa.blk_per_problem;
+__global__ __launch_bounds__(256, 1) void potrf_diag128_slim(StepArgs sa, RiderArgs ra) {
+    const int prob = (int)blockIdx.x;
+    if (blockIdx.y != 0) { draw_rider(ra, (int)blockIdx.y - 1, prob, (int)threadIdx.x); return; }
+    sa.S += (int64_t)prob * sa.pS;
+    sa.L += (int64_t)prob * sa.pL;
+    sa.X += (int64_t)prob * sa.pX;
+    sa.blk += prob * sa.blk_per_problem;
     extern __shared__ __attribute__((aligned(16))) double smem[];
     double* Ts = smem;
     double* Xs = Ts + TILE_ELEMS;
diff --git a/diffeqgmrfs.jl_amd/posterior.py b/diffeqgmrfs.jl_amd/posterior.py
--- a/diffeqgmrfs.jl_amd/posterior.py
+++ b/diffeqgmrfs.jl_amd/posterior.py
@@ -234,7 +234,12 @@
         self.timing = timing and hasattr(engine, "torch")
         self._ev = None
 
+    def _register_draws(self, first: int):
+        if self.replicate and type(self.e) is HipEngine and getattr(self.e, "batch", 1) > 1 and self.k <= 128:
+            self.e.F.set_factor_draws(self.k, self.seed, first)
+
     def prepare(self):
+        self._register_draws(self.rank * self.k * getattr(self.e, "batch", 1))
         self.e.prepare(is_root=(self.rank == 0), shared_storage=not self.replicate, dist=self.dist)
         if self.dist is not None and self.world > 1:
             self.dist.barrier()
@@ -275,9 +280,10 @@
             self.e.adopt_commit()
 
     def step(self, step_index: int = 0):
-        self._factor_and_share()
         nb = getattr(self.e, "batch", 1)
         first = (step_index * self.world + self.rank) * self.k * nb
+        self._register_draws(first)
+        self._factor_and_share()
         if self.replicate and type(self.e) is HipEngine:
             mu, X = self.e.posterior(self.k, self.seed, first, keep=self.keep_samples)
         else:
diff --git a/include/gmrf_hip.h b/include/gmrf_hip.h
--- a/include/gmrf_hip.h
+++ b/include/gmrf_hip.h
@@ -56,6 +56,7 @@
     int32_t persist_refused;
     int32_t sweep_persist;
     int32_t sweep_persist_launches;
+    int32_t posterior_draws_in_factor;
 } gmrf_stats;
 
 
@@ -86,6 +87,8 @@
                               double* mean, double* samples, int64_t ld);
 
 gmrf_status gmrf_bt_set_factor_rhs(gmrf_handle* h, const double* b);
+
+gmrf_status gmrf_bt_set_factor_draws(gmrf_handle* h, int64_t k, uint64_t seed, int64_t first_id);
 
 gmrf_status gmrf_bt_normals(gmrf_handle* h, uint64_t seed, int64_t first_id, int64_t k,
                             double* z, int64_t ld);
@@ -316,6 +319,8 @@
                                   double* S, double* L, double* Linv, int32_t* info, int32_t* route);
 gmrf_status gmrf_test_persist_stamps(double* out, int32_t n);
 gmrf_status gmrf_test_persist_aborts(gmrf_handle* h, int32_t* n);
+gmrf_status gmrf_test_drawn_panel(gmrf_handle* h, int64_t* k, double* out);
+gmrf_status gmrf_test_draw_slice(uint64_t T, uint64_t S, uint64_t s, uint64_t* first);
 gmrf_status gmrf_test_factor_fwd(gmrf_handle* h, int32_t* state, double* y_out);
 gmrf_status gmrf_test_gn_route(gmrf_gn* g, int32_t* iterations, int32_t* fwd_iterations);
 gmrf_status gmrf_test_dc_route(gmrf_dc* g, int32_t* fwd_in_factor);
```

Measured after the change: 54570 solves/s (median of 6 runs). Within noise of the previous version (+0.8%).
